# PythonOptimizers/pysparse

Measured on AMD Instinct MI355X. Metric: CSR SpMV GB/s (7-pt Poisson, % of 8 TB/s HBM peak) + PCG iters/s, higher is better.
Workload: dtype f64

## Files before the change

### include/pysparse_hip.h

```cpp
#ifndef PYSPARSE_HIP_H
#define PYSPARSE_HIP_H

#include <stddef.h>
#include <stdint.h>

#ifdef __cplusplus
extern "C" {
#endif

#define PSP_OK 0
#define PSP_EINVAL (-1)
#define PSP_ENODEV (-2)
#define PSP_ENOMEM (-3)
#define PSP_ESINGULAR (-4)
#define PSP_ECALLBACK (-5)

#define PSP_INFO_CONVERGED 0
#define PSP_INFO_MAXIT (-1)
#define PSP_INFO_ILLCOND_PRECON (-2)
#define PSP_INFO_NOT_SPD_PRECON (-3)
#define PSP_INFO_STAGNATION (-5)
#define PSP_INFO_BREAKDOWN (-6)

typedef struct psp_csr psp_csr_t;
// ... 1 lines not shown
typedef struct psp_jacobi psp_jacobi_t;
typedef struct psp_ssor psp_ssor_t;
typedef struct psp_op psp_op_t;


const char *psp_last_error(void);
const char *psp_version(void);
int psp_device_count(void);
int psp_set_device(int device);
int psp_thread_info(int *thread_slot, int *device, void **hip_stream);
int psp_debug_hold_handles(const void *h1, const void *h2, int milliseconds);
int psp_debug_mid_count(long long *solves, long long *fallbacks);
int psp_debug_brick_count(long long *solves, long long *fallbacks);
int psp_debug_shake(long long seed, int min_us, int max_us, unsigned point_mask, unsigned rank_mask, int revert_mask);
int psp_debug_shake_count(long long *injected);
int psp_debug_spin(int microseconds);
int psp_peer_access(int device, int peer, int *can_access);
int psp_set_placement(int on);
int psp_placement_info(int *enabled, long long *draws, double *draw_ms_total);
int psp_place_operands(const psp_csr_t *A, double **y_dev, double **x_dev, double *report6);
int psp_set_stream(void *hip_stream);
int psp_synchronize(void);
int psp_device_info(char *name, int name_len, int *compute_units, int64_t *hbm_bytes);
int psp_mem_info(int64_t *free_bytes, int64_t *total_bytes);

int psp_malloc(void **dev, size_t bytes);
int psp_free(void *dev);
int psp_memcpy_h2d(void *dev, const void *host, size_t bytes);
int psp_memcpy_d2h(void *host, const void *dev, size_t bytes);
int psp_memset(void *dev, int byte, size_t bytes);
int psp_trim(void);
int psp_event_create(void **event);
int psp_event_destroy(void *event);
int psp_event_record(void *event);
int psp_event_elapsed_ms(void *start, void *stop, float *ms);
int psp_stream_probe(int reads, int writes, size_t bytes_per_stream, int reps, float *avg_ms, float *min_ms);
int psp_last_solve_info(char *name, int name_cap, int *info);
int psp_set_single_kernel_loops(int on);
const char *psp_build_id(void);


int psp_csr_create(int nrows, int ncols, int nnz, const int *ind_host, const int *col_host,
                   const double *val_host, psp_csr_t **out);
int psp_csr_poisson(int nx, int ny, int nz, psp_csr_t **out);
int psp_csr_poisson_slab(int nx, int ny, int nz, int64_t row_lo, int64_t row_hi, int64_t col_shift,
                         int ncols_local, psp_csr_t **out);
int psp_csr_poisson_big(int nx, int ny, int nz, psp_csr_t **out);
int psp_csr_poisson_big_slab(int nx, int ny, int nz, int64_t row_lo, int64_t row_hi, int64_t col_shift,
                             int ncols_local, psp_csr_t **out);
int64_t psp_csr_nnz64(const psp_csr_t *A);
int psp_csr_poisson_multi(int nx, int ny, int nz, const int *devices, int ndev, psp_csr_t **out);
int psp_csr_create_multi(int nrows, int ncols, int nnz, const int *ind_host, const int *col_host,
                         const double *val_host, const int *devices, int ndev, psp_csr_t **out);
int psp_csr_multi_info(const psp_csr_t *A, int *nranks, int *distinct_devices, int *uses_rccl);
int psp_multi_plan(int nrows, int ncols, const int *ind_host, const int *col_host, int ndev, int rank,
                   int64_t *row_range_out, int *counts_out, int *ghost_ids, int ghost_cap, int *links, int links_cap,
                   int *col_local);
int psp_csr_multi_spmv_time(psp_csr_t *A, int warmup, int reps, double *ms_per_product);
int psp_csr_multi_phase_time(psp_csr_t *A, int what, int warmup, int reps, double *ms_per_rep);
int psp_csr_create64(int nrows, int ncols, int64_t nnz, const int64_t *ind_host, const int *col_host,
                     const double *val_host, psp_csr_t **out);
int psp_csr_random_banded(int nrows, int ncols, int m, int stride, uint64_t seed, psp_csr_t **out);
int psp_csr_download_rows(const psp_csr_t *A, int row_lo, int row_hi, int64_t *ind_host, int *col_host,
                          double *val_host);
int psp_csr_destroy(psp_csr_t *A);
int psp_csr_shape(const psp_csr_t *A, int *nrows, int *ncols, int *nnz);
int psp_csr_download(const psp_csr_t *A, int *ind_host, int *col_host, double *val_host);
int psp_csr_diagonal(const psp_csr_t *A, double *diag_host);

int psp_csr_matvec(psp_csr_t *A, const double *x_host, double *y_host);
int psp_csr_matvec_stride(psp_csr_t *A, const double *x_host, ptrdiff_t incx, double *y_host,
                          ptrdiff_t incy);
int psp_csr_matvec_transp(psp_csr_t *A, const double *x_host, double *y_host);
int psp_csr_matvec_transp_stride(psp_csr_t *A, const double *x_host, ptrdiff_t incx,
                                 double *y_host, ptrdiff_t incy);
int psp_csr_matvec_dev(psp_csr_t *A, const double *x_dev, double *y_dev);
int psp_csr_matvec_transp_dev(psp_csr_t *A, const double *x_dev, double *y_dev);
int psp_csr_set_variant(psp_csr_t *A, int variant);
int psp_csr_set_schedule(psp_csr_t *A, int strip_rows);
int psp_csr_kernel_info(psp_csr_t *A, char *name, int name_cap, int *info);
int psp_csr_prepare(psp_csr_t *A, long long expected_products);
int psp_csr_release_arrays(psp_csr_t *A);
int psp_csr_setup_info(psp_csr_t *A, double *info4);
int psp_csr_renumbering(psp_csr_t *A, int *perm_host, int *available);
int64_t psp_csr_device_bytes(const psp_csr_t *A);


int psp_sss_create(int n, int nnz_lower, const int *ind_host, const int *col_host,
                   const double *val_host, const double *diag_host, psp_sss_t **out);
int psp_sss_poisson(int nx, int ny, int nz, psp_sss_t **out);
int psp_sss_destroy(psp_sss_t *A);
int psp_sss_kernel_info(psp_sss_t *A, char *name, int name_cap, int *info);
int psp_sss_prepare(psp_sss_t *A, long long expected_products);
int psp_sss_setup_info(psp_sss_t *A, double *info4);
int psp_sss_set_variant(psp_sss_t *A, int variant);
int psp_sss_shape(const psp_sss_t *A, int *n, int *nnz_reported);
int psp_sss_download(const psp_sss_t *A, int *ind_host, int *col_host, double *val_host,
                     double *diag_host);
int psp_sss_getitem(const psp_sss_t *A, int i, int j, double *value);
int psp_sss_matvec(psp_sss_t *A, const double *x_host, double *y_host);
int psp_sss_matvec_stride(psp_sss_t *A, const double *x_host, ptrdiff_t incx, double *y_host,
                          ptrdiff_t incy);
int psp_sss_matvec_dev(psp_sss_t *A, const double *x_dev, double *y_dev);
int64_t psp_sss_device_bytes(const psp_sss_t *A);


int psp_jacobi_create_csr(psp_csr_t *A, double omega, int steps, psp_jacobi_t **out);
int psp_jacobi_create_sss(psp_sss_t *A, double omega, int steps, psp_jacobi_t **out);
int psp_jacobi_create_diag(int n, const double *diag_host, double omega, int steps,
                           const psp_op_t *A_or_null, psp_jacobi_t **out);
int psp_jacobi_destroy(psp_jacobi_t *K);
int psp_jacobi_shape(const psp_jacobi_t *K, int *n);
int psp_jacobi_precon(psp_jacobi_t *K, const double *x_host, double *y_host);
int psp_jacobi_precon_dev(psp_jacobi_t *K, const double *x_dev, double *y_dev);


int psp_ssor_create(psp_sss_t *A, double omega, int steps, psp_ssor_t **out);
int psp_ssor_destroy(psp_ssor_t *K);
int psp_ssor_info(const psp_ssor_t *K, int *n, int *levels_forward, int *levels_backward);
int psp_ssor_run_info(const psp_ssor_t *K, int *runs_forward, int *runs_backward, long *levels_in_runs,
                      long *slots_in_runs);
int psp_ssor_brick_info(const psp_ssor_t *K, int *bricks, int *edge);
int psp_ssor_precon(psp_ssor_t *K, const double *x_host, double *y_host);
int psp_ssor_precon_dev(psp_ssor_t *K, const double *x_dev, double *y_dev);


typedef int (*psp_host_apply_fn)(void *ctx, int n, const double *x_host, double *y_host);

int psp_op_from_csr(psp_csr_t *A, psp_op_t **out);
int psp_op_from_sss(psp_sss_t *A, psp_op_t **out);
int psp_op_from_jacobi(psp_jacobi_t *K, psp_op_t **out);
int psp_op_from_ssor(psp_ssor_t *K, psp_op_t **out);
int psp_op_from_callback(int n, psp_host_apply_fn fn, void *ctx, psp_op_t **out);
int psp_op_destroy(psp_op_t *op);


int psp_pcg(const psp_op_t *A, const psp_op_t *K, int n, double *x_host, const double *b_host,
            double tol, int maxit, int *info, int *iter, double *relres, double *hist_host);
int psp_pcg_dev(const psp_op_t *A, const psp_op_t *K, int n, double *x_dev, const double *b_dev,
                double tol, int maxit, int *info, int *iter, double *relres, double *hist_host);

int psp_minres(const psp_op_t *A, const psp_op_t *K, int n, double *x_host, const double *b_host,
               double tol, int maxit, int *info, int *iter, double *relres, double *hist_host);
int psp_minres_dev(const psp_op_t *A, const psp_op_t *K, int n, double *x_dev,
                   const double *b_dev, double tol, int maxit, int *info, int *iter,
                   double *relres, double *hist_host);

int psp_cgs(const psp_op_t *A, const psp_op_t *K, int n, double *x_host, const double *b_host,
            double tol, int maxit, int *info, int *iter, double *relres);
int psp_bicgstab(const psp_op_t *A, const psp_op_t *K, int n, double *x_host, const double *b_host,
                 double tol, int maxit, int *info, int *iter, double *relres);
int psp_qmrs(const psp_op_t *A, const psp_op_t *K, int n, double *x_host, const double *b_host,
             double tol, int maxit, int *info, int *iter, double *relres);
int psp_gmres(const psp_op_t *A, const psp_op_t *K, int n, double *x_host, const double *b_host,
              double tol, int maxit, int dim, int *info, int *iter, double *relres);


int psp_k_hint_constant(const double *v_dev, int n);
int psp_k_unhint(const double *v_dev);
int psp_k_dot(int n, const double *x_dev, const double *y_dev, double *out_dev);
int psp_k_residual(int n, const double *b_dev, double *r_dev, const double *dinv_dev,
                   double *out_dev);
int psp_k_pupdate(int n, const double *r_dev, const double *dinv_dev, double beta, int first,
                  double *p_dev);
int psp_k_csr_matvec_dot(psp_csr_t *A, const double *p_dev, int p_offset, double *q_dev,
                         double *out_dev);
// ... 67 lines not shown
```

### pysparse_amd/_capi.py

```python
import ctypes as C
import os

HERE = os.path.dirname(os.path.abspath(__file__))
LIB_PATH = os.environ.get("PSP_LIB_OVERRIDE") or os.path.join(HERE, "libpysparse_hip.so")

SYMBOLS = """
psp_last_error psp_version psp_device_count psp_set_device psp_thread_info psp_debug_hold_handles psp_debug_mid_count psp_debug_brick_count psp_debug_shake psp_debug_shake_count psp_debug_spin psp_peer_access psp_set_stream psp_synchronize
psp_set_placement psp_placement_info psp_place_operands psp_device_info psp_mem_info psp_malloc psp_free psp_memcpy_h2d psp_memcpy_d2h psp_memset psp_trim
psp_event_create psp_event_destroy psp_event_record psp_event_elapsed_ms psp_stream_probe psp_build_id psp_last_solve_info psp_set_single_kernel_loops
psp_csr_create psp_csr_poisson psp_csr_poisson_slab psp_csr_poisson_big psp_csr_poisson_big_slab psp_csr_nnz64 psp_csr_create64 psp_csr_random_banded psp_csr_download_rows psp_csr_destroy psp_csr_shape
psp_csr_download psp_csr_diagonal psp_csr_matvec psp_csr_matvec_stride psp_csr_matvec_transp
psp_csr_matvec_transp_stride psp_csr_matvec_dev psp_csr_matvec_transp_dev psp_csr_set_variant
psp_csr_set_schedule psp_csr_kernel_info psp_csr_prepare psp_csr_setup_info psp_csr_release_arrays psp_csr_renumbering psp_csr_device_bytes
psp_csr_poisson_multi psp_csr_create_multi psp_csr_multi_info psp_csr_multi_spmv_time psp_csr_multi_phase_time psp_multi_plan
psp_sss_create psp_sss_poisson psp_sss_destroy psp_sss_shape psp_sss_download psp_sss_getitem
psp_sss_matvec psp_sss_matvec_stride psp_sss_matvec_dev psp_sss_device_bytes
psp_sss_kernel_info psp_sss_set_variant psp_sss_prepare psp_sss_setup_info
psp_jacobi_create_csr psp_jacobi_create_sss psp_jacobi_create_diag psp_jacobi_destroy
psp_jacobi_shape psp_jacobi_precon psp_jacobi_precon_dev
psp_ssor_create psp_ssor_destroy psp_ssor_info psp_ssor_run_info psp_ssor_brick_info psp_ssor_precon psp_ssor_precon_dev
psp_op_from_csr psp_op_from_sss psp_op_from_jacobi psp_op_from_ssor psp_op_from_callback psp_op_destroy
psp_pcg psp_pcg_dev psp_minres psp_minres_dev psp_cgs psp_bicgstab psp_qmrs psp_gmres
psp_k_dot psp_k_residual psp_k_pupdate psp_k_csr_matvec_dot psp_k_xr_update psp_k_gather
psp_k_csr_matvec_overlap psp_k_hint_constant psp_k_unhint psp_k_px_update psp_k_r_update psp_k_x_update
psp_k_jacobi psp_pcgstate_create psp_pcgstate_destroy psp_pcgstate_init psp_pcgstate_fetch psp_pcgstate_hist
psp_kd_px_update psp_kd_csr_matvec_overlap psp_kd_pcg_scalar_xpq psp_kd_r_update psp_kd_pcg_scalar_r
psp_minresstate_create psp_minresstate_destroy psp_minresstate_init psp_minresstate_fetch psp_minresstate_hist
psp_kd_minres_scale psp_kd_minres_matvec psp_kd_minres_lanczos psp_kd_minres_scalar psp_kd_minres_wx
""".split()


class PcgStatus(C.Structure):
    _fields_ = [("status", C.c_int), ("info", C.c_int), ("iter", C.c_int), ("it", C.c_int), ("xpend", C.c_int),
                ("stag0", C.c_int), ("pend_maxit", C.c_int), ("relres", C.c_double), ("normr", C.c_double),
                ("n2b", C.c_double), ("alpha_x", C.c_double)]


class MinresStatus(C.Structure):
    _fields_ = [("status", C.c_int), ("stop", C.c_int), ("info", C.c_int), ("iter", C.c_int),
                ("relres", C.c_double), ("norm_rmr", C.c_double)]

WAIT_FN = C.CFUNCTYPE(C.c_int, C.c_void_p)
HOST_APPLY_FN = C.CFUNCTYPE(C.c_int, C.c_void_p, C.c_int, C.POINTER(C.c_double), C.POINTER(C.c_double))


class PspError(RuntimeError):
    def __init__(self, code, msg):
        RuntimeError.__init__(self, "libpysparse_hip error %d: %s" % (code, msg))
        self.code = code


_lib = None


def lib():
    global _lib
    if _lib is None:
        if not os.path.exists(LIB_PATH):
            raise ImportError("%s not found: run `python -c 'import __graft_entry__ as g; g.build()'` "
                              "(hipcc --offload-arch=gfx950); there is no CPU fallback" % LIB_PATH)
        L = C.CDLL(LIB_PATH)
        _declare(L)
        _lib = L
    return _lib


def check(rc):
    if rc != 0:
        raise PspError(rc, lib().psp_last_error().decode())
    return rc


def _declare(L):
    vp, i, d, i64 = C.c_void_p, C.c_int, C.c_double, C.c_int64
    pvp, pi, pd = C.POINTER(C.c_void_p), C.POINTER(C.c_int), C.POINTER(C.c_double)
    sz, pt = C.c_size_t, C.c_ssize_t
    L.psp_last_error.restype = C.c_char_p
    L.psp_last_error.argtypes = []
    L.psp_version.restype = C.c_char_p
    L.psp_version.argtypes = []
    L.psp_device_count.restype = i
    L.psp_device_count.argtypes = []
    sig = {
        "psp_set_device": [i], "psp_thread_info": [pi, pi, pvp], "psp_debug_hold_handles": [vp, vp, i], "psp_debug_shake": [C.c_longlong, i, i, C.c_uint, C.c_uint, i], "psp_debug_shake_count": [C.POINTER(C.c_longlong)], "psp_debug_spin": [i], "psp_debug_mid_count": [C.POINTER(C.c_longlong), C.POINTER(C.c_longlong)], "psp_debug_brick_count": [C.POINTER(C.c_longlong), C.POINTER(C.c_longlong)], "psp_peer_access": [i, i, pi], "psp_set_stream": [vp], "psp_synchronize": [], "psp_trim": [],
        "psp_set_placement": [i], "psp_placement_info": [pi, C.POINTER(C.c_longlong), pd], "psp_place_operands": [vp, pvp, pvp, pd],
        "psp_device_info": [C.c_char_p, i, pi, C.POINTER(i64)],
        "psp_mem_info": [C.POINTER(i64), C.POINTER(i64)],
        "psp_malloc": [pvp, sz], "psp_free": [vp], "psp_memcpy_h2d": [vp, vp, sz],
        "psp_memcpy_d2h": [vp, vp, sz], "psp_memset": [vp, i, sz],
        "psp_event_create": [pvp], "psp_event_destroy": [vp], "psp_event_record": [vp],
        "psp_event_elapsed_ms": [vp, vp, C.POINTER(C.c_float)],
        "psp_stream_probe": [i, i, sz, i, C.POINTER(C.c_float), C.POINTER(C.c_float)],
        "psp_csr_create": [i, i, i, vp, vp, vp, pvp],
        "psp_csr_poisson": [i, i, i, pvp], "psp_csr_poisson_big": [i, i, i, pvp],
        "psp_csr_poisson_slab": [i, i, i, i64, i64, i64, i, pvp],
        "psp_csr_poisson_big_slab": [i, i, i, i64, i64, i64, i, pvp],
        "psp_csr_create64": [i, i, i64, vp, vp, vp, pvp],
        "psp_csr_poisson_multi": [i, i, i, vp, i, pvp], "psp_csr_create_multi": [i, i, i, vp, vp, vp, vp, i, pvp],
        "psp_csr_multi_info": [vp, pi, pi, pi], "psp_csr_multi_spmv_time": [vp, i, i, pd], "psp_csr_multi_phase_time": [vp, i, i, i, pd],
        "psp_multi_plan": [i, i, vp, vp, i, i, C.POINTER(i64), vp, vp, i, vp, i, vp],
        "psp_csr_random_banded": [i, i, i, i, C.c_uint64, pvp],
        "psp_csr_download_rows": [vp, i, i, vp, vp, vp],
        "psp_csr_destroy": [vp], "psp_csr_shape": [vp, pi, pi, pi],
        "psp_csr_download": [vp, vp, vp, vp], "psp_csr_diagonal": [vp, vp],
        "psp_csr_matvec": [vp, vp, vp], "psp_csr_matvec_stride": [vp, vp, pt, vp, pt],
        "psp_csr_matvec_transp": [vp, vp, vp], "psp_csr_matvec_transp_stride": [vp, vp, pt, vp, pt],
        "psp_csr_matvec_dev": [vp, vp, vp], "psp_csr_matvec_transp_dev": [vp, vp, vp],
        "psp_csr_set_variant": [vp, i], "psp_csr_set_schedule": [vp, i],
        "psp_csr_kernel_info": [vp, C.c_char_p, i, pi],
        "psp_csr_renumbering": [vp, vp, pi],
        "psp_sss_create": [i, i, vp, vp, vp, vp, pvp], "psp_sss_poisson": [i, i, i, pvp],
        "psp_sss_destroy": [vp], "psp_sss_shape": [vp, pi, pi],
        "psp_sss_download": [vp, vp, vp, vp, vp], "psp_sss_getitem": [vp, i, i, pd],
        "psp_sss_matvec": [vp, vp, vp], "psp_sss_matvec_stride": [vp, vp, pt, vp, pt],
        "psp_sss_matvec_dev": [vp, vp, vp],
        "psp_sss_kernel_info": [vp, C.c_char_p, i, pi], "psp_sss_set_variant": [vp, i],
        "psp_jacobi_create_csr": [vp, d, i, pvp], "psp_jacobi_create_sss": [vp, d, i, pvp],
        "psp_jacobi_create_diag": [i, vp, d, i, vp, pvp], "psp_jacobi_destroy": [vp],
        "psp_jacobi_shape": [vp, pi], "psp_jacobi_precon": [vp, vp, vp],
        "psp_jacobi_precon_dev": [vp, vp, vp],
        "psp_ssor_create": [vp, d, i, pvp], "psp_ssor_destroy": [vp], "psp_ssor_info": [vp, pi, pi, pi], "psp_ssor_run_info": [vp, pi, pi, vp, vp], "psp_ssor_brick_info": [vp, pi, pi],
        "psp_ssor_precon": [vp, vp, vp], "psp_ssor_precon_dev": [vp, vp, vp], "psp_op_from_ssor": [vp, pvp],
        "psp_op_from_csr": [vp, pvp], "psp_op_from_sss": [vp, pvp], "psp_op_from_jacobi": [vp, pvp],
        "psp_op_from_callback": [i, HOST_APPLY_FN, vp, pvp], "psp_op_destroy": [vp],
        "psp_pcg": [vp, vp, i, vp, vp, d, i, pi, pi, pd, vp],
        "psp_pcg_dev": [vp, vp, i, vp, vp, d, i, pi, pi, pd, vp],
        "psp_minres": [vp, vp, i, vp, vp, d, i, pi, pi, pd, vp],
        "psp_minres_dev": [vp, vp, i, vp, vp, d, i, pi, pi, pd, vp],
        "psp_cgs": [vp, vp, i, vp, vp, d, i, pi, pi, pd], "psp_bicgstab": [vp, vp, i, vp, vp, d, i, pi, pi, pd],
        "psp_qmrs": [vp, vp, i, vp, vp, d, i, pi, pi, pd], "psp_gmres": [vp, vp, i, vp, vp, d, i, i, pi, pi, pd],
        "psp_k_dot": [i, vp, vp, vp], "psp_k_residual": [i, vp, vp, vp, vp],
        "psp_k_pupdate": [i, vp, vp, d, i, vp], "psp_k_csr_matvec_dot": [vp, vp, i, vp, vp],
        "psp_k_xr_update": [i, d, vp, vp, vp, vp, vp, vp], "psp_k_gather": [i, vp, vp, vp],
        "psp_k_csr_matvec_overlap": [vp, vp, i, vp, i, i, WAIT_FN, vp, vp],
        "psp_k_hint_constant": [vp, i], "psp_k_unhint": [vp],
        "psp_k_px_update": [i, vp, vp, d, i, d, i, vp, vp, vp], "psp_k_r_update": [i, d, vp, vp, vp, vp],
        "psp_k_x_update": [i, d, vp, vp, vp],
        "psp_k_jacobi": [i, vp, vp, vp],
        "psp_pcgstate_create": [pvp], "psp_pcgstate_destroy": [vp], "psp_pcgstate_init": [vp, d, d, d, d, i, i],
        "psp_pcgstate_fetch": [vp, C.POINTER(PcgStatus)], "psp_pcgstate_hist": [vp, i, i, vp],
        "psp_kd_px_update": [vp, i, vp, vp, vp, vp, vp],
        "psp_kd_csr_matvec_overlap": [vp, vp, vp, i, vp, i, i, WAIT_FN, vp, vp],
        "psp_kd_pcg_scalar_xpq": [vp, vp], "psp_kd_r_update": [vp, i, vp, vp, vp, vp],
        "psp_kd_pcg_scalar_r": [vp, vp],
        "psp_minresstate_create": [pvp], "psp_minresstate_destroy": [vp],
        "psp_minresstate_init": [vp, d, d, d, i, i], "psp_minresstate_fetch": [vp, C.POINTER(MinresStatus)],
        "psp_minresstate_hist": [vp, i, i, vp],
        "psp_kd_minres_scale": [vp, i, vp, vp],
        "psp_kd_minres_matvec": [vp, vp, vp, i, vp, i, i, WAIT_FN, vp, vp],
        "psp_kd_minres_lanczos": [vp, i, vp, vp, vp, vp, vp, vp], "psp_kd_minres_scalar": [vp, i, vp],
        "psp_kd_minres_wx": [vp, i, vp, vp, vp, vp],
        "psp_last_solve_info": [C.c_char_p, i, C.POINTER(i)], "psp_set_single_kernel_loops": [i],
        "psp_csr_release_arrays": [vp], "psp_csr_prepare": [vp, C.c_longlong], "psp_sss_prepare": [vp, C.c_longlong],
        "psp_csr_setup_info": [vp, C.POINTER(d)], "psp_sss_setup_info": [vp, C.POINTER(d)],
    }
    for name, argtypes in sig.items():
        f = getattr(L, name)
        f.restype = i
        f.argtypes = argtypes
    L.psp_build_id.restype = C.c_char_p
    L.psp_build_id.argtypes = []
    L.psp_csr_device_bytes.restype = i64
    L.psp_csr_device_bytes.argtypes = [vp]
    L.psp_csr_nnz64.restype = i64
    L.psp_csr_nnz64.argtypes = [vp]
    L.psp_sss_device_bytes.restype = i64
    L.psp_sss_device_bytes.argtypes = [vp]
```

### pysparse_amd/csrc/psp_csr_abi.h

```cpp

__global__ __launch_bounds__(256) void csr_validate_kernel(int nnz, int ncols, const int *__restrict__ col,
                                                           unsigned long long *bad) {
  for (long k = (long)blockIdx.x * 256 + threadIdx.x; k < nnz; k += (long)gridDim.x * 256) {
    const int c = col[k];
    if (c < 0 || c >= ncols) atomicMin(bad, (unsigned long long)k);
  }
}

extern "C" {

int psp_csr_create(int nrows, int ncols, int nnz, const int *ind_host, const int *col_host,
                   const double *val_host, psp_csr_t **out) {
  if (psp::cpu_mode()) return psp::cpu::csr_create(nrows, ncols, nnz, ind_host, col_host, val_host, out);
  if (!out || !ind_host || (nnz > 0 && (!col_host || !val_host)))
    return fail(PSP_EINVAL, "psp_csr_create: NULL argument");
  if (nrows < 0 || ncols < 0 || nnz < 0) return fail(PSP_EINVAL, "psp_csr_create: negative size");
  if (ind_host[0] != 0 || ind_host[nrows] != nnz)
    return fail(PSP_EINVAL, "psp_csr_create: ind[0] must be 0 and ind[nrows] == nnz");
  for (int i = 0; i < nrows; ++i)
    if (ind_host[i + 1] < ind_host[i])
      return fail(PSP_EINVAL, "psp_csr_create: ind not monotone at row %d", i);
  const bool check_on_device = nnz >= (1 << 22);
  if (!check_on_device)
    for (int k = 0; k < nnz; ++k)
// ... 231 lines not shown
    if (rc == PSP_OK) rc = finalize_csr(P);
    if (rc != PSP_OK) {
      if (P) psp_csr_destroy(P);
      if (A) psp_csr_destroy(A);
      return rc;
    }
    if (!A) {
      *out = P;
      return PSP_OK;
    }
    P->no_reorder = true;
    A->parts[p] = P;
    A->part_row0[p] = (int)r0;
    A->max_row_nnz = std::max(A->max_row_nnz, P->max_row_nnz);
  }
  A->part_row0[np] = nrows;
  *out = A;
  return PSP_OK;
}

int psp_csr_download_rows(const psp_csr_t *A, int row_lo, int row_hi, int64_t *ind_host, int *col_host,
                          double *val_host) {
  if (A && A->multi) return fail(PSP_EINVAL, "%s is not available on a multi-device matrix (psp_csr_*_multi): use matvec, jacobi, pcg, minres", "psp_csr_download_rows");
  if (!A || !ind_host) return fail(PSP_EINVAL, "psp_csr_download_rows: NULL argument");
  if (A->w4_only) return fail(PSP_EINVAL, "psp_csr_download_rows: the operator has no CSR arrays (psp_csr_poisson_big, psp_csr_release_arrays)");
  if (row_lo < 0 || row_hi > A->nrows || row_lo > row_hi) return fail(PSP_EINVAL, "psp_csr_download_rows: bad row range");
  int64_t written = 0;
  ind_host[0] = 0;
  const int np = A->nparts ? A->nparts : 1;
  for (int p = 0; p < np; ++p) {
    const psp_csr *P = A->nparts ? A->parts[p] : A;
    const int p0 = A->nparts ? A->part_row0[p] : 0;
    const int a = std::max(row_lo, p0) - p0, b = std::min(row_hi, p0 + P->nrows) - p0;
    if (a >= b) continue;
    std::vector<int> pi((size_t)(b - a) + 1);
    PSP_HIP(hipMemcpy(pi.data(), P->ind + a, sizeof(int) * pi.size(), hipMemcpyDeviceToHost));
    const int k0 = pi[0], cnt = pi.back() - k0;
    for (int r = a; r < b; ++r) ind_host[(size_t)(p0 + r - row_lo) + 1] = written + (pi[(size_t)(r - a) + 1] - k0);
    if (cnt > 0) {
      if (col_host) PSP_HIP(hipMemcpy(col_host + written, P->col + k0, sizeof(int) * (size_t)cnt, hipMemcpyDeviceToHost));
      if (val_host) PSP_HIP(hipMemcpy(val_host + written, P->val + k0, sizeof(double) * (size_t)cnt, hipMemcpyDeviceToHost));
    }
    written += cnt;
  }
  return PSP_OK;
}

int psp_csr_destroy(psp_csr_t *A) {
  if (!A) return PSP_OK;
  if (A->host) return psp::cpu::csr_destroy(A);
  if (A->multi) {
    PSP_API_GUARD_H(A);
    const int rc = psp::multi_destroy(A->multi);
    delete A;
    return rc;
  }
  psp_csr *transposed = nullptr, *reordered = nullptr;
  {
    std::lock_guard<std::mutex> lk(g_extra_mu);
    auto it = g_extra.find(A);
    if (it != g_extra.end()) {
      transposed = it->second.transposed;
      reordered = it->second.reordered;
      if (it->second.perm) (void)hipFree(it->second.perm);
      if (it->second.inv) (void)hipFree(it->second.inv);
      if (it->second.xp) (void)hipFree(it->second.xp);
      for (auto &t : it->second.t) {
        if (t.second.tab) (void)hipFree(t.second.tab);
        if (t.second.rowoff) (void)hipFree(t.second.rowoff);
        if (t.second.blist) (void)hipFree(t.second.blist);
        if (t.second.blist6) (void)hipFree(t.second.blist6);
        if (t.second.col16) (void)hipFree(t.second.col16);
        if (t.second.ulist) (void)hipFree(t.second.ulist);
        if (t.second.colu) (void)hipFree(t.second.colu);
        if (t.second.perm) (void)hipFree(t.second.perm);
      }
      if (it->second.big_partials) (void)hipFree(it->second.big_partials);
      if (it->second.packed) (void)hipFree(it->second.packed);
      if (it->second.dia_val) (void)hipFree(it->second.dia_val);
      if (it->second.dia_mask) (void)hipFree(it->second.dia_mask);
      if (it->second.dia_mask32) (void)hipFree(it->second.dia_mask32);
      if (it->second.dia_mask64) (void)hipFree(it->second.dia_mask64);
      if (it->second.dia_offs_dev) (void)hipFree(it->second.dia_offs_dev);
      g_extra.erase(it);
    }
  }
  for (int p = 0; p < A->nparts; ++p) psp_csr_destroy(A->parts[p]);
  delete[] A->parts;
  delete[] A->part_row0;
  if (transposed) psp_csr_destroy(transposed);
  if (reordered) psp_csr_destroy(reordered);
  (void)hipFree(A->ind);
  (void)hipFree(A->col);
  (void)hipFree(A->val);
  delete A;
  return PSP_OK;
}

int psp_csr_shape(const psp_csr_t *A, int *nrows, int *ncols, int *nnz) {
  if (!A) return fail(PSP_EINVAL, "psp_csr_shape: NULL handle");
  if (nrows) *nrows = A->nrows;
  if (ncols) *ncols = A->ncols;
  if (nnz) *nnz = A->nnz;
  return PSP_OK;
}

int psp_csr_download(const psp_csr_t *A, int *ind_host, int *col_host, double *val_host) {
  if (A && A->host) return psp::cpu::csr_download(A, ind_host, col_host, val_host);
  if (A && A->multi) return fail(PSP_EINVAL, "%s is not available on a multi-device matrix (psp_csr_*_multi): use matvec, jacobi, pcg, minres", "psp_csr_download");
  if (!A) return fail(PSP_EINVAL, "psp_csr_download: NULL handle");
  if (A->w4_only) return fail(PSP_EINVAL, "psp_csr_download: the operator has no CSR arrays (psp_csr_poisson_big, psp_csr_release_arrays)");
  if (A->nparts) return fail(PSP_EINVAL, "psp_csr_download: more than 2^31 nonzeros: use psp_csr_download_rows");
  if (ind_host)
    PSP_HIP(hipMemcpyAsync(ind_host, A->ind, sizeof(int) * ((size_t)A->nrows + 1),
                           hipMemcpyDeviceToHost, stream()));
  if (col_host && A->nnz)
    PSP_HIP(hipMemcpyAsync(col_host, A->col, sizeof(int) * (size_t)A->nnz, hipMemcpyDeviceToHost,
                           stream()));
  if (val_host && A->nnz)
    PSP_HIP(hipMemcpyAsync(val_host, A->val, sizeof(double) * (size_t)A->nnz,
                           hipMemcpyDeviceToHost, stream()));
  PSP_HIP(hipStreamSynchronize(stream()));
  return PSP_OK;
}

int psp_csr_diagonal_dev(const psp_csr_t *A, double *diag_dev) {
  PSP_API_GUARD_H(A);
  if (A && A->multi) return fail(PSP_EINVAL, "%s is not available on a multi-device matrix (psp_csr_*_multi): use matvec, jacobi, pcg, minres", "psp_csr_diagonal_dev");
  if (A->nrows == 0) return PSP_OK;
  if (A->nparts) {
    for (int p = 0; p < A->nparts; ++p) {
      const psp_csr *P = A->parts[p];
      if (P->nrows == 0) continue;
      hipLaunchKernelGGL(csr_diag_kernel, dim3(std::min((P->nrows + 255) / 256, 4096)), dim3(256), 0, stream(),
                         P->nrows, A->part_row0[p], P->ind, P->col, P->val, diag_dev + A->part_row0[p]);
    }
    PSP_LAUNCH_CHECK();
    return PSP_OK;
  }
  if (A->w4_only) {
    psp::CsrExtra *ex;
    PSP_TRY(ensure_w4(A, &ex));
    const int zero_slot = A->w4_diag_slot;
    hipLaunchKernelGGL(dia_diag_kernel, dim3(std::min((A->nrows + 255) / 256, 65536)), dim3(256), 0, stream(),
                       A->nrows, ex->dia_no, zero_slot, ex->dia_val, ex->dia_mask, diag_dev);
    PSP_LAUNCH_CHECK();
    return PSP_OK;
  }
  int grid = std::min((A->nrows + 255) / 256, 4096);
  hipLaunchKernelGGL(csr_diag_kernel, dim3(grid), dim3(256), 0, stream(), A->nrows, 0, A->ind, A->col,
                     A->val, diag_dev);
  PSP_LAUNCH_CHECK();
  return PSP_OK;
}

int psp_csr_diagonal(const psp_csr_t *A, double *diag_host) {
  PSP_API_GUARD_H(A);
  if (!A || !diag_host) return fail(PSP_EINVAL, "psp_csr_diagonal: NULL argument");
  if (A->host) return psp::cpu::csr_diagonal(A, diag_host);
  if (A->multi) return psp::multi_diagonal_host(A->multi, diag_host);
  DevBuf d;
  PSP_TRY(d.alloc(A->nrows));
  PSP_TRY(psp_csr_diagonal_dev(A, d.p));
  return download_strided(diag_host, d.p, A->nrows, 1);
}

// ... 96 lines not shown
      dperm = it->second.perm;
      on_device = it->second.reorder_on_device;
    }
  }
  if (!dperm) return PSP_OK;
  PSP_HIP(hipMemcpy(perm_host, dperm, sizeof(int) * (size_t)A->nrows, hipMemcpyDeviceToHost));
  *available = on_device ? 2 : 1;
  return PSP_OK;
}

int psp_csr_release_arrays(psp_csr_t *A) {
  PSP_API_GUARD_H(A);
  if (!A) return fail(PSP_EINVAL, "psp_csr_release_arrays: NULL handle");
  if (A->w4_only) return PSP_OK;
  if (A->host || A->multi || A->nparts || A->sym_owner)
    return fail(PSP_EINVAL, "psp_csr_release_arrays: not available for this kind of handle");
  PSP_TRY(ensure_device());
  psp::CsrExtra *ex;
  PSP_TRY(ensure_w4(A, &ex));
  if (ex->dia_state != 1 || ex->dia_no > 16)
    return fail(PSP_EINVAL, "psp_csr_release_arrays: the operator does not multiply with the index-free layout (csr_spmv_w4, "
                            "<= 16 offsets): its CSR arrays are what it streams");
  PSP_HIP(hipStreamSynchronize(stream()));
  int slot = -1;
  for (int o = 0; o < ex->dia_no; ++o)
    if (ex->dia_offs.o[o] == 0) slot = o;
  psp_csr *transposed = nullptr, *reordered = nullptr;
  {
    std::lock_guard<std::mutex> lk(g_extra_mu);
    transposed = ex->transposed;
    reordered = ex->reordered;
    ex->transposed = ex->reordered = nullptr;
    for (auto &t : ex->t) {
      if (t.second.tab) (void)hipFree(t.second.tab);
      if (t.second.rowoff) (void)hipFree(t.second.rowoff);
      if (t.second.blist) (void)hipFree(t.second.blist);
      if (t.second.blist6) (void)hipFree(t.second.blist6);
      if (t.second.col16) (void)hipFree(t.second.col16);
      if (t.second.ulist) (void)hipFree(t.second.ulist);
      if (t.second.colu) (void)hipFree(t.second.colu);
      if (t.second.perm) (void)hipFree(t.second.perm);
    }
    ex->t.clear();
    if (ex->packed) (void)hipFree(ex->packed);
    ex->packed = nullptr;
  }
  if (transposed) psp_csr_destroy(transposed);
  if (reordered) psp_csr_destroy(reordered);
  if (A->ind) (void)hipFree(A->ind);
  if (A->col) (void)hipFree(A->col);
  if (A->val) (void)hipFree(A->val);
  A->ind = A->col = nullptr;
  A->val = nullptr;
  A->padded = 0;
  A->nnz64 = A->nnz;
  A->w4_diag_slot = slot;
  A->max_row_nnz = ex->dia_no;
  A->variant = -1;
  A->w4_only = true;
  return PSP_OK;
}

int psp_csr_prepare(psp_csr_t *A, long long expected_products) {
  PSP_API_GUARD_H(A);
  if (!A) return fail(PSP_EINVAL, "psp_csr_prepare: NULL handle");
  if (A->host || A->multi || A->nparts) return PSP_OK;
  std::lock_guard<std::mutex> lk(g_extra_mu);
  g_extra[A].expected_products = expected_products < 0 ? 0 : (expected_products > 0x7fffffffffffLL ? 0x7fffffffffffLL : (long)expected_products);
  return PSP_OK;
}

int psp_csr_setup_info(psp_csr_t *A, double *info4) {
  PSP_API_GUARD_H(A);
  if (!A || !info4) return fail(PSP_EINVAL, "psp_csr_setup_info: NULL argument");
  info4[0] = info4[1] = info4[2] = info4[3] = 0.0;
  if (A->host || A->multi || A->nparts) return PSP_OK;
  std::lock_guard<std::mutex> lk(g_extra_mu);
  auto it = g_extra.find(A);
  if (it == g_extra.end()) return PSP_OK;
  info4[0] = it->second.reorder_ms;
  info4[1] = (double)it->second.products;
  info4[2] = (double)reorder_after();
  info4[3] = (double)it->second.reorder_state;
  return PSP_OK;
}

int psp_csr_kernel_info(psp_csr_t *A, char *name, int name_cap, int *info) {
  PSP_API_GUARD_H(A);
  if (!A) return fail(PSP_EINVAL, "psp_csr_kernel_info: NULL handle");
  if (A->host) {
    if (name && name_cap > 0) snprintf(name, name_cap, "cpu loops (PSP_DEVICE=cpu)");
    if (info) info[0] = info[1] = info[2] = info[3] = 0;
    return PSP_OK;
  }
  if (A->multi) {
    char buf[160];
    psp::multi_describe(A->multi, buf, sizeof buf);
    if (name && name_cap > 0) snprintf(name, name_cap, "%s", buf);
    if (info) info[0] = info[1] = info[2] = info[3] = 0;
    return PSP_OK;
  }
  if (A->nparts) return psp_csr_kernel_info(A->parts[0], name, name_cap, info);
  Variant v = decode_variant(A->variant);
  if (A->w4_only) v.w4 = true;
  const char *k = "csr_spmv_stream";
  int vals[4] = {0, 0, 0, 0};
  bool w4 = false;
  if (v.w4 && A->sym_owner) {
    psp_sss *S = const_cast<psp_sss *>(A->sym_owner);
    PSP_TRY(ensure_sss_w4(S));
    if (S->w4_state == 1) {
      w4 = true;
      k = "sss_spmv_w4";
      vals[0] = S->w4_nol;
    }
  }
  if (!w4 && v.w4) {
    psp::CsrExtra *ex;
    PSP_TRY(ensure_w4(A, &ex));
    if (ex->dia_state == 1) {
      w4 = true;
      k = "csr_spmv_w4";
      vals[0] = ex->dia_no;
    }
  }
  if (!w4 && A->nrows > 0 && (v.wave || v.w1) && A->max_row_nnz <= v.tile / 2) {
    k = v.wave ? "csr_spmv_wave" : "csr_spmv_w1";
    if (v.w2) {
      ChunkTable *t;
      PSP_TRY(get_chunk_table(A, v.tile, &t));
      PSP_TRY(ensure_rowoff(A, t));
      if (t->np != 0) {
        k = "csr_spmv_w2";
        if (v.w3) {
          PSP_TRY(ensure_w3(A, t));
          vals[1] = t->max_blocks;
          {
            psp::CsrExtra *exs = nullptr;
            int mode = 0;
            PSP_TRY(pick_scattered(A, t, &exs, &mode));
            if (mode == 1) {
              ChunkTable *rt;
              PSP_TRY(get_chunk_table(exs->reordered, 1024, &rt));
              k = "csr_spmv_w3_rcm";
              vals[0] = rt->nb;
              vals[1] = rt->max_blocks;
              vals[3] = t->max_blocks;
            } else if (mode == 2) {
              k = "csr_spmv_w5";
              vals[0] = t->nu;
              vals[3] = t->max_cols;
            }
          }
          if (t->nb > 0) {
            k = "csr_spmv_w3";
            vals[0] = t->nb;
            if (v.sched) {
              PSP_TRY(ensure_schedule(A, t));
              vals[2] = t->sched_state == 1;
              vals[3] = t->half_band;
            }
          }
        }
        if (v.w6 && !strcmp(k, "csr_spmv_w2")) {
          PSP_TRY(ensure_w6(A, t));
          if (t->nb6 > 0) {
// ... 351 lines not shown
```

### pysparse_amd/csrc/psp_csr_kernels.h

```cpp

constexpr int kBlock = 256;


__global__ void build_chunk_table(int nrows, const int *__restrict__ ind, int target, int nchunks,
                                  int2 *__restrict__ tab) {
  int c = blockIdx.x * blockDim.x + threadIdx.x;
  if (c > nchunks) return;
  int r;
  if (c == nchunks) {
    r = nrows;
  } else {
    long want = (long)c * target;
    int lo = 0, hi = nrows;
    while (lo < hi) {
      int mid = lo + ((hi - lo) >> 1);
      if ((long)ind[mid] >= want)
        hi = mid;
      else
        lo = mid + 1;
    }
    r = lo;
  }
  tab[c] = make_int2(r, ind[r]);
}
// ... 1255 lines not shown
      if constexpr (NTS)
        __builtin_nontemporal_store(outu, reinterpret_cast<d2u *>(y + r));
      else
        *reinterpret_cast<d2u *>(y + r) = outu;
      if (dotv) {
        d2u u;
        if (dot_slot >= 0) {
          u.x = 0.0;
          u.y = 0.0;
#pragma unroll
          for (int o = 0; o < NO; ++o)
            if (o == dot_slot) {
              u.x = xv[o].x;
              u.y = xv[o].y;
            }
        } else {
          u = *reinterpret_cast<const d2u *>(dotv + r);
          if (use_div) {
            u.x = u.x / xdiv;
            u.y = u.y / xdiv;
          }
        }
        dsum += u.x * a0;
        dsum += u.y * a1;
      }
    } else {
      y[r] = a0;
      if (dotv) {
        double u0 = 0.0;
        if (dot_slot >= 0) {
#pragma unroll
          for (int o = 0; o < NO; ++o)
            if (o == dot_slot) u0 = xv[o].x;
        } else {
          u0 = use_div ? dotv[r] / xdiv : dotv[r];
        }
        dsum += u0 * a0;
      }
    }
  }
  if (partials) {
    dsum = wave_sum(dsum);
    if (lane == 0) red[wid] = dsum;
    __syncthreads();
    if (threadIdx.x == 0) partials[blockIdx.x] = red[0] + red[1] + red[2] + red[3];
  }
}

struct SssOffs {
  int o[8];
};

__global__ void sss_lowmask_kernel(int n, int nol, SssOffs offs, const int *__restrict__ ind,
                                   const int *__restrict__ col, const double *__restrict__ val,
                                   double *__restrict__ valL, unsigned char *__restrict__ low, long soa_npad) {
  for (long r = (long)blockIdx.x * blockDim.x + threadIdx.x; r < n; r += (long)gridDim.x * blockDim.x) {
    const long blk = r / kDiaRows;
    const int i = (int)(r % kDiaRows);
    unsigned m = 0;
    for (int k = ind[r]; k < ind[r + 1]; ++k) {
      const int o = col[k] - (int)r;
      int b = 0;
      while (b < nol - 1 && offs.o[b] != o) ++b;
      m |= 1u << b;
      if (soa_npad > 0) valL[(size_t)b * soa_npad + r] = val[k];
      else valL[((size_t)blk * nol + b) * kDiaRows + i] = val[k];
    }
    low[r] = (unsigned char)m;
  }
}

__global__ void sss_mask_kernel(int n, int nol, SssOffs offs, const unsigned char *__restrict__ low,
                                unsigned short *__restrict__ mask) {
  for (long r = (long)blockIdx.x * blockDim.x + threadIdx.x; r < n; r += (long)gridDim.x * blockDim.x) {
    unsigned m = low[r];
    for (int j = 0; j < nol; ++j) {
      const long ru = r - offs.o[j];
      if (ru < n && ((low[ru] >> j) & 1u)) m |= 1u << (8 + j);
    }
    mask[r] = (unsigned short)m;
  }
}

template <int NOL, int FLAGS = 0>
__global__ __launch_bounds__(256) void sss_spmv_w4(
    int n, int stripe, SssOffs offs, const double *__restrict__ valL, const double *__restrict__ diag,
    const unsigned short *__restrict__ mask, const double *__restrict__ x, double *__restrict__ y,
    const double *__restrict__ dotv, double *__restrict__ partials, const int *__restrict__ skip,
    int use_div, double xdiv, const double *__restrict__ xdiv_dev, int dot_is_x) {
  if (skip && *skip) return;
  if (xdiv_dev) xdiv = *xdiv_dev;
  __shared__ double red[4];
  const int lane = threadIdx.x & 63;
  const int wid = __builtin_amdgcn_readfirstlane(threadIdx.x >> 6);
  int vb = (int)blockIdx.x;
  if (stripe > 0) {
    const int k = vb >> 3;
    vb = ((k / stripe) * 8 + (vb & 7)) * stripe + k % stripe;
  }
  const long blk = (long)vb * 4 + wid;
  const long r = blk * kDiaRows + 2 * lane;
  double dsum = 0.0;
  if (r < n) {
    const bool two = r + 1 < n;
    const unsigned mm = *reinterpret_cast<const unsigned *>(mask + r);
    const unsigned m0 = mm & 0xffffu, m1 = mm >> 16;
    const long npad = ((long)n + kDiaRows - 1) / kDiaRows * kDiaRows;
    const long xmax = (long)n - 2;
    bool edge = !two;
    constexpr bool SOA = (FLAGS & 8) != 0;
    auto vaddr = [&](long row, int j) -> const double * {
      return SOA ? valL + (size_t)j * npad + row
                 : valL + ((size_t)(row / kDiaRows) * NOL + j) * kDiaRows + (size_t)(row % kDiaRows);
    };
    d2v vl[NOL], xl[NOL];
    constexpr bool SHFL = (FLAGS & 4) != 0;
    const bool off1 = SHFL && offs.o[NOL - 1] == -1;
#pragma unroll
    for (int j = 0; j < NOL; ++j) {
      vl[j] = ldg<(FLAGS & 1) != 0>(reinterpret_cast<const d2v *>(vaddr(r, j)));
      if (off1 && j == NOL - 1) continue;
      const long c = r + offs.o[j];
      const long cc = c < 0 ? 0 : c;
      const d2u t = *reinterpret_cast<const d2u *>(x + cc);
      xl[j].x = t.x;
      xl[j].y = t.y;
      edge |= c < 0;
    }
    double halo_xm1 = 0.0, halo_x2 = 0.0, halo_v2 = 0.0;
    if (off1) {
      if (lane == 0 && r > 0) halo_xm1 = x[r - 1];
      if (lane == 63) {
        if (r + 2 < n) halo_x2 = x[r + 2];
        if (r + 2 < npad)
          halo_v2 = *vaddr(r + 2, NOL - 1);
      }
    }
    d2v dg, x0;
    {
      const long rd = r > xmax ? xmax : r;
      const d2u t = *reinterpret_cast<const d2u *>(diag + rd);
      const d2u u = *reinterpret_cast<const d2u *>(x + rd);
      dg.x = t.x; dg.y = t.y; x0.x = u.x; x0.y = u.y;
    }
    d2v vu[NOL], xu[NOL];
#pragma unroll
    for (int j = 0; j < NOL; ++j) {
      if (off1 && j == NOL - 1) continue;
      const long ru = r - offs.o[j];
      if (SHFL && (offs.o[j] & 1) == 0) {
        const long v0 = ru < npad ? ru : npad - 2;
        vu[j] = ldg<(FLAGS & 2) != 0>(reinterpret_cast<const d2v *>(vaddr(v0, j)));
      } else {
        const long v0 = ru < npad ? ru : npad - 1, v1 = ru + 1 < npad ? ru + 1 : npad - 1;
        vu[j].x = ldg<(FLAGS & 2) != 0>(vaddr(v0, j));
        vu[j].y = ldg<(FLAGS & 2) != 0>(vaddr(v1, j));
      }
      const long xr = ru > xmax ? xmax : ru;
      const d2u t = *reinterpret_cast<const d2u *>(x + xr);
      xu[j].x = t.x;
      xu[j].y = t.y;
      edge |= ru > xmax;
    }
    if (edge) {
#pragma unroll
      for (int j = 0; j < NOL; ++j) {
        const long c = r + offs.o[j];
        if (c < 0) {
          xl[j].x = 0.0;
          xl[j].y = c + 1 >= 0 ? x[c + 1] : 0.0;
        }
        const long ru = r - offs.o[j];
        if (ru > xmax) {
          xu[j].x = ru < n ? x[ru] : 0.0;
          xu[j].y = 0.0;
        }
      }
      if (!two) {
        dg.x = diag[r];
        dg.y = 0.0;
        x0.x = x[r];
        x0.y = 0.0;
      }
    }
    if (off1) {
      constexpr int j = NOL - 1;
      const double up = __shfl_up(x0.y, 1, 64);
      const double dnx = __shfl_down(x0.x, 1, 64);
      const double dnv = __shfl_down(vl[j].x, 1, 64);
      xl[j].x = lane == 0 ? halo_xm1 : up;
      xl[j].y = x0.x;
      vu[j].x = vl[j].y;
      vu[j].y = lane == 63 ? halo_v2 : dnv;
      xu[j].x = x0.y;
      xu[j].y = lane == 63 ? halo_x2 : dnx;
    }
    if (use_div) {
#pragma unroll
      for (int j = 0; j < NOL; ++j) {
        xl[j].x = xl[j].x / xdiv;
        xl[j].y = xl[j].y / xdiv;
        xu[j].x = xu[j].x / xdiv;
        xu[j].y = xu[j].y / xdiv;
      }
      x0.x = x0.x / xdiv;
      x0.y = x0.y / xdiv;
    }
    double a0 = 0.0, a1 = 0.0;
#pragma unroll
    for (int j = 0; j < NOL; ++j) {
      const double t0 = a0 + vl[j].x * xl[j].x;
      const double t1 = a1 + vl[j].y * xl[j].y;
      a0 = ((m0 >> j) & 1u) ? t0 : a0;
      a1 = ((m1 >> j) & 1u) ? t1 : a1;
    }
    a0 = a0 + dg.x * x0.x;
    a1 = a1 + dg.y * x0.y;
#pragma unroll
    for (int j = NOL - 1; j >= 0; --j) {
      const double t0 = a0 + vu[j].x * xu[j].x;
      const double t1 = a1 + vu[j].y * xu[j].y;
      a0 = ((m0 >> (8 + j)) & 1u) ? t0 : a0;
      a1 = ((m1 >> (8 + j)) & 1u) ? t1 : a1;
    }
    if (two) {
      d2u outu;
      outu.x = a0;
      outu.y = a1;
      __builtin_nontemporal_store(outu, reinterpret_cast<d2u *>(y + r));
      if (dotv) {
        d2u u;
        if (dot_is_x) {
          u.x = x0.x;
          u.y = x0.y;
        } else {
          u = *reinterpret_cast<const d2u *>(dotv + r);
          if (use_div) {
            u.x = u.x / xdiv;
            u.y = u.y / xdiv;
          }
        }
        dsum += u.x * a0;
        dsum += u.y * a1;
      }
    } else {
      y[r] = a0;
      if (dotv) dsum += (dot_is_x ? x0.x : (use_div ? dotv[r] / xdiv : dotv[r])) * a0;
    }
  }
  if (partials) {
    dsum = wave_sum(dsum);
    if (lane == 0) red[wid] = dsum;
    __syncthreads();
    if (threadIdx.x == 0) partials[blockIdx.x] = red[0] + red[1] + red[2] + red[3];
  }
}

template <int NO>
__global__ __launch_bounds__(256) void csr_spmv_w4x(
    int blk0, int blk1, int nrows, int ncols, int stripe, DiaOffs offs, const double *__restrict__ valT,
    const unsigned *__restrict__ mask, const double *__restrict__ x, double *__restrict__ y,
    const double *__restrict__ dotv, double *__restrict__ partials, const int *__restrict__ skip) {
  if (skip && *skip) return;
  __shared__ double red[4];
  const int lane = threadIdx.x & 63;
  const int wid = __builtin_amdgcn_readfirstlane(threadIdx.x >> 6);
  int vb = (int)blockIdx.x;
  if (stripe > 0) {
    const int k = vb >> 3;
    vb = ((k / stripe) * 8 + (vb & 7)) * stripe + k % stripe;
  }
  const int blk = blk0 + vb * 4 + wid;
  const long r = (long)blk * kDiaRows + 2 * lane;
  double dsum = 0.0;
  if (blk < blk1 && r < nrows) {
    const uint2 mm = *reinterpret_cast<const uint2 *>(mask + r);
    const unsigned m0 = mm.x, m1 = mm.y;
    const double *vp = valT + (size_t)blk * NO * kDiaRows + 2 * lane;
    const long cmax = (long)ncols - 2;
    double a0 = 0.0, a1 = 0.0;
#pragma unroll
    for (int g = 0; g < NO; g += 8) {
      constexpr int G = 8;
      d2v v[G], xv[G];
      bool edge = false;
#pragma unroll
      for (int u = 0; u < G; ++u) {
        if (g + u < NO) {
          v[u] = ldg<true>(reinterpret_cast<const d2v *>(vp + (g + u) * kDiaRows));
          const long c = r + offs.o[g + u];
          const long cc = c < 0 ? 0 : (c > cmax ? cmax : c);
          const d2u t = *reinterpret_cast<const d2u *>(x + cc);
          xv[u].x = t.x;
          xv[u].y = t.y;
          edge |= cc != c;
        }
      }
      if (edge) {
#pragma unroll
        for (int u = 0; u < G; ++u) {
          if (g + u < NO) {
            const long c = r + offs.o[g + u];
            if (c < 0 || c > cmax) {
              xv[u].x = (c >= 0 && c < ncols) ? x[c] : 0.0;
              xv[u].y = (c + 1 >= 0 && c + 1 < ncols) ? x[c + 1] : 0.0;
            }
          }
        }
      }
#pragma unroll
      for (int u = 0; u < G; ++u) {
        if (g + u < NO) {
          const double t0 = a0 + v[u].x * xv[u].x;
          const double t1 = a1 + v[u].y * xv[u].y;
          a0 = ((m0 >> (g + u)) & 1u) ? t0 : a0;
          a1 = ((m1 >> (g + u)) & 1u) ? t1 : a1;
        }
      }
    }
    if (r + 1 < nrows) {
      d2u outu;
      outu.x = a0;
      outu.y = a1;
      __builtin_nontemporal_store(outu, reinterpret_cast<d2u *>(y + r));
      if (dotv) {
        const d2u u = *reinterpret_cast<const d2u *>(dotv + r);
        dsum += u.x * a0;
        dsum += u.y * a1;
      }
    } else {
      y[r] = a0;
      if (dotv) dsum += dotv[r] * a0;
    }
  }
  if (partials) {
    dsum = wave_sum(dsum);
    if (lane == 0) red[wid] = dsum;
// ... 415 lines not shown
```

### pysparse_amd/csrc/psp_csr_select.h

```cpp
namespace psp {

static int colmask() {
#ifdef PSP_TUNING
  static const int m = [] {
    const char *e = psp::tuning_env("PSP_SPMV_COLMASK");
    return e ? atoi(e) : -1;
  }();
  return m;
#else
  return -1;
#endif
}

static int spmv_stripe() {
  static const int m = [] {
    const char *e = psp::tuning_env("PSP_SPMV_STRIPE");
    return e ? atoi(e) : -1;
  }();
  return m;
}

static int w4_auto_stripe(const psp_csr *A) {
  if (A->sym_owner) return 32;
  int plane_wgs = 0;
// ... 94 lines not shown
}

static void launch_w5(const psp_csr *A, const ChunkTable *t, int grid, int stripe, int c0, int c1, const double *x,
                      double *y, const double *dotv, double *pbuf, const int *skip) {
  if (t->np == 2) launch_w5_np<2>(A, t, grid, stripe, c0, c1, x, y, dotv, pbuf, skip);
  else if (t->np == 3) launch_w5_np<3>(A, t, grid, stripe, c0, c1, x, y, dotv, pbuf, skip);
  else launch_w5_np<4>(A, t, grid, stripe, c0, c1, x, y, dotv, pbuf, skip);
}

constexpr long kReorderAfter = 2048;
static long reorder_after() {
  static const long v = [] {
    const char *e = psp::tuning_env("PSP_SPMV_REORDER_AFTER");
    return e ? atol(e) : kReorderAfter;
  }();
  return v;
}

static int pick_scattered(const psp_csr *A, ChunkTable *t, psp::CsrExtra **ex_out, int *mode, bool count = false) {
  *mode = 0;
  if (t->nb != 0 || t->max_blocks <= 0) return PSP_OK;
  const int var = A->variant < 0 ? 0 : A->variant;
  if (((var >> 27) & 1) == 0) {
    psp::CsrExtra *exr;
    bool due;
    {
      std::lock_guard<std::mutex> lk(g_extra_mu);
      exr = &g_extra[A];
      due = exr->reorder_state >= 0 || exr->products >= reorder_after() || exr->expected_products >= reorder_after();
      if (count && !due) exr->products += 1;
    }
    if (due) {
      PSP_TRY(ensure_reordered(A, exr, t->max_blocks));
      if (exr->reorder_state == 1) {
        *ex_out = exr;
        *mode = 1;
        return PSP_OK;
      }
    }
  }
  if (((var >> 28) & 1) == 0) {
    PSP_TRY(ensure_w5(A, t));
    if (t->nu > 0) *mode = 2;
  }
  return PSP_OK;
}

static int launch_reordered(const psp_csr *A, psp::CsrExtra *ex, int stripe, const double *x, double *y,
                            const double *dotv, double *partials, int *nparts, const int *skip) {
  psp_csr *R = ex->reordered;
  ChunkTable *t;
  PSP_TRY(get_chunk_table(R, 1024, &t));
  int grid = (t->nchunks + 3) / 4;
  if (stripe > 0) grid = (grid + 8 * stripe - 1) / (8 * stripe) * (8 * stripe);
  const int n = A->nrows;
  double *xp = ex->xp, *yp = ex->xp + n;
  static const bool gather_form = [] {
    const char *e = psp::tuning_env("PSP_SPMV_REORDER_GATHER");
    return e && atoi(e) != 0;
  }();
  if (gather_form) PSP_TRY(psp::reorder_gather(n, ex->perm, x, xp, skip));
  else PSP_TRY(psp::reorder_scatter(n, ex->inv, x, xp, skip));
  R->variant = A->variant;
  launch_w3(R, t, true, grid, stripe, 0, t->nchunks, xp, yp, nullptr, nullptr, skip);
  PSP_LAUNCH_CHECK();
  const int gback = (n + 1023) / 1024;
  double *pbuf = partials;
  if (partials && gback > kMaxParts) {
    PSP_TRY(ensure_big_partials(ex, gback));
    pbuf = ex->big_partials;
  }
  int np = 0;
  if (!partials && !gather_form) PSP_TRY(psp::reorder_scatter(n, ex->perm, yp, y, skip));
  else PSP_TRY(psp::reorder_back(n, ex->inv, yp, y, partials ? dotv : nullptr, pbuf, &np, skip));
  if (partials && pbuf != partials) {
    hipLaunchKernelGGL(fold_partials_kernel, dim3(kFold / 16), dim3(256), 0, stream(), pbuf, np, partials, kFold);
    PSP_LAUNCH_CHECK();
    np = kFold;
  }
  if (nparts) *nparts = np;
  return PSP_OK;
}

int csr_spmv_scaled_launch(const psp_csr *A, const double *x, double xdiv, double *y, double *partials,
                           int *nparts, int *available, const int *skip, const double *xdiv_dev) {
  *available = 0;
  static const bool on = [] {
    const char *e = psp::tuning_env("PSP_MINRES_SCALED");
    return e ? atoi(e) != 0 : true;
  }();
  Variant v = decode_variant(A->variant);
  if (A->w4_only) v.w4 = true;
  if (!on || !v.w4 || A->nparts || A->nrows != A->ncols || A->nrows < 2) return PSP_OK;
  const int stripe = w4_stripe(A, v);
  const int nblk = (A->nrows + kDiaRows - 1) / kDiaRows;
  const int grid = w4_grid(nblk, stripe);
  psp::CsrExtra *ex;
  {
    std::lock_guard<std::mutex> lk(g_extra_mu);
    ex = &g_extra[A];
  }
  bool sss = false;
  if (A->sym_owner) {
    psp_sss *S = const_cast<psp_sss *>(A->sym_owner);
    PSP_TRY(ensure_sss_w4(S));
    sss = S->w4_state == 1;
  }
  if (!sss) {
    PSP_TRY(ensure_w4(A, &ex));
    if (ex->dia_state != 1 || ex->dia_no > 16) return PSP_OK;
  }
  double *pbuf = partials;
  if (partials && grid > kMaxParts) {
    PSP_TRY(ensure_big_partials(ex, grid));
    pbuf = ex->big_partials;
  }
  if (sss)
    PSP_TRY(launch_sss_w4(A->sym_owner, stripe, x, y, x, pbuf, skip, grid, 1, xdiv, xdiv_dev));
  else
    PSP_TRY(launch_w4(A, ex, stripe, 0, nblk, x, y, x, pbuf, skip, grid, 1, xdiv, xdiv_dev));
  int np = grid;
  if (pbuf != partials) {
    np = kFold;
    hipLaunchKernelGGL(fold_partials_kernel, dim3(np / 16), dim3(256), 0, stream(), pbuf, grid, partials, np);
    PSP_LAUNCH_CHECK();
  }
  if (nparts) *nparts = np;
  *available = 1;
  return PSP_OK;
}

__global__ __launch_bounds__(256) void grid_wrap_check_kernel(int n, int nx, int ny, const unsigned short *__restrict__ mask,
                                                              int *__restrict__ bad) {
  int found = 0;
  for (long r = (long)blockIdx.x * blockDim.x + threadIdx.x; r < n; r += (long)gridDim.x * blockDim.x) {
    const unsigned m = mask[r];
    const int i = (int)(r % nx), j = (int)((r / nx) % ny);
    if (((m >> 2) & 1u) && i == 0) found = 1;
    if (((m >> 4) & 1u) && i == nx - 1) found = 1;
    if (((m >> 1) & 1u) && j == 0) found = 1;
    if (((m >> 5) & 1u) && j == ny - 1) found = 1;
  }
  if (found) atomicAdd(bad, 1);
}

__global__ __launch_bounds__(256) void w4_value_range_kernel(int n, int no, const double *__restrict__ valT,
                                                             const unsigned short *__restrict__ mask, double *__restrict__ out) {
  __shared__ double smin[4][16], smax[4][16];
  double lo[16], hi[16];
  for (int o = 0; o < 16; ++o) {
    lo[o] = INFINITY;
    hi[o] = -INFINITY;
  }
  for (long r = (long)blockIdx.x * blockDim.x + threadIdx.x; r < n; r += (long)gridDim.x * blockDim.x) {
    const unsigned m = mask[r];
    const double *vp = valT + (size_t)(r / kDiaRows) * no * kDiaRows + (size_t)(r % kDiaRows);
    for (int o = 0; o < no; ++o)
      if ((m >> o) & 1u) {
        const double v = vp[(size_t)o * kDiaRows];
        lo[o] = v < lo[o] ? v : lo[o];
        hi[o] = v > hi[o] ? v : hi[o];
        if (!(v == v)) hi[o] = INFINITY, lo[o] = -INFINITY;
      }
  }
  const int lane = threadIdx.x & 63, wid = threadIdx.x >> 6;
  for (int o = 0; o < no; ++o) {
    double a = lo[o], b = hi[o];
    for (int off = 32; off > 0; off >>= 1) {
      const double a2 = __shfl_down(a, off, 64), b2 = __shfl_down(b, off, 64);
      a = a2 < a ? a2 : a;
      b = b2 > b ? b2 : b;
    }
    if (lane == 0) {
      smin[wid][o] = a;
      smax[wid][o] = b;
    }
  }
  __syncthreads();
  if ((int)threadIdx.x < no) {
    const int o = threadIdx.x;
    double a = smin[0][o], b = smax[0][o];
    for (int w = 1; w < 4; ++w) {
      a = smin[w][o] < a ? smin[w][o] : a;
      b = smax[w][o] > b ? smax[w][o] : b;
    }
    out[((size_t)blockIdx.x * no + o) * 2] = a;
    out[((size_t)blockIdx.x * no + o) * 2 + 1] = b;
  }
}

int csr_w4_view(const psp_csr *A, W4View *out, int *available) {
  *available = 0;
  Variant v = decode_variant(A->variant);
  if (A->w4_only) v.w4 = true;
  if (!v.w4 || A->nparts || A->multi || A->host || A->nrows != A->ncols || A->nrows < 2) return PSP_OK;
  psp::CsrExtra *ex;
  PSP_TRY(ensure_w4(A, &ex));
  if (ex->dia_state != 1 || ex->dia_no > 9 || !ex->dia_mask) return PSP_OK;
  out->no = ex->dia_no;
  for (int i = 0; i < 12; ++i) out->offs[i] = i < ex->dia_no ? ex->dia_offs.o[i] : 0;
  out->valT = ex->dia_val;
// ... 179 lines not shown
  return t->np != 0;
}

int csr_reordered_view(const psp_csr *A, psp_csr **R, const int **perm, const int **inv) {
  *R = nullptr;
  psp::setup_mark(nullptr);
  Variant v = decode_variant(A->variant);
  if (A->nparts || A->w4_only || A->no_reorder || !(v.w1 && v.w2 && v.w3) || A->nrows != A->ncols ||
      A->max_row_nnz > v.tile / 2 || v.tile != 1024)
    return PSP_OK;
  if (v.w4) {
    if (A->sym_owner) {
      psp_sss *S = const_cast<psp_sss *>(A->sym_owner);
      PSP_TRY(ensure_sss_w4(S));
      if (S->w4_state == 1) return PSP_OK;
    }
    psp::CsrExtra *ex;
    PSP_TRY(ensure_w4(A, &ex));
    if (ex->dia_state == 1) return PSP_OK;
  }
  psp::setup_mark("first use: index-free (w4) layouts tried");
  ChunkTable *t;
  PSP_TRY(get_chunk_table(const_cast<psp_csr *>(A), v.tile, &t));
  PSP_TRY(ensure_rowoff(A, t));
  if (t->np == 0) return PSP_OK;
  psp::setup_mark("first use: chunk table + row offsets");
  PSP_TRY(ensure_w3(A, t));
  psp::setup_mark("first use: w3 tables on the stored numbering");
  psp::CsrExtra *exs = nullptr;
  int mode = 0;
  PSP_TRY(pick_scattered(A, t, &exs, &mode));
  if (mode != 1) return PSP_OK;
  exs->reordered->variant = A->variant;
  *R = exs->reordered;
  *perm = exs->perm;
  *inv = exs->inv;
  return PSP_OK;
}

int csr_spmv_launch(const psp_csr *A, const double *x, double *y, const double *dotv,
                    double *partials, int *nparts, const int *skip) {
  Workspace *w;
  PSP_TRY(workspace(&w));
  psp::setup_mark(nullptr);
  if (A->nparts) {
    double *tmp = w->partials + (size_t)(kSlots - 1) * kMaxParts;
    if (partials && (partials == tmp || (long)A->nparts * kFold > kMaxParts))
      return fail(PSP_EINVAL, "csr_spmv_launch: partitioned matrix needs a partial-sum slot other than the last");
    for (int p = 0; p < A->nparts; ++p) {
      const psp_csr *P = A->parts[p];
      if (P->nrows == 0) continue;
      const int r0 = A->part_row0[p];
      int np = 0;
      PSP_TRY(csr_spmv_launch(P, x, y + r0, (partials && dotv) ? dotv + r0 : nullptr, partials ? tmp : nullptr, &np,
                              skip));
      if (partials) {
        hipLaunchKernelGGL(fold_partials_kernel, dim3(kFold / 16), dim3(256), 0, stream(), tmp, np,
                           partials + (size_t)p * kFold, kFold);
        PSP_LAUNCH_CHECK();
      }
    }
    if (nparts) *nparts = A->nparts * kFold;
    return PSP_OK;
  }
  Variant v = decode_variant(A->variant);
  if (A->w4_only) v.w4 = true;
  if (v.w4 && A->sym_owner) {
    psp_sss *S = const_cast<psp_sss *>(A->sym_owner);
    PSP_TRY(ensure_sss_w4(S));
    if (S->w4_state == 1) {
      const int stripe = w4_stripe(A, v);
      const int nblk = (S->n + kDiaRows - 1) / kDiaRows;
      const int grid = w4_grid(nblk, stripe);
      double *pbuf = partials;
      if (partials && grid > kMaxParts) {
        psp::CsrExtra *ex;
        {
          std::lock_guard<std::mutex> lk(g_extra_mu);
          ex = &g_extra[A];
        }
        PSP_TRY(ensure_big_partials(ex, grid));
        pbuf = ex->big_partials;
      }
      PSP_TRY(launch_sss_w4(S, stripe, x, y, dotv, pbuf, skip, grid));
      int np = grid;
      if (pbuf != partials) {
        np = kFold;
        hipLaunchKernelGGL(fold_partials_kernel, dim3(np / 16), dim3(256), 0, stream(), pbuf, grid,
                           partials, np);
        PSP_LAUNCH_CHECK();
      }
      if (nparts) *nparts = np;
      return PSP_OK;
    }
  }
  if (v.w4) {
    psp::CsrExtra *ex;
    PSP_TRY(ensure_w4(A, &ex));
    if (ex->dia_state == 1) {
      const int stripe = w4_stripe(A, v);
      const int nblk = (A->nrows + kDiaRows - 1) / kDiaRows;
      const int grid = w4_grid(nblk, stripe);
      double *pbuf = partials;
      if (partials && grid > kMaxParts) {
        PSP_TRY(ensure_big_partials(ex, grid));
        pbuf = ex->big_partials;
      }
      PSP_TRY(launch_w4(A, ex, stripe, 0, nblk, x, y, dotv, pbuf, skip, grid));
      int np = grid;
      if (pbuf != partials) {
        np = kFold;
        hipLaunchKernelGGL(fold_partials_kernel, dim3(np / 16), dim3(256), 0, stream(), pbuf, grid,
                           partials, np);
        PSP_LAUNCH_CHECK();
      }
      if (nparts) *nparts = np;
      return PSP_OK;
    }
  }
  if (A->w4_only) return fail(PSP_EINVAL, "this operator exists only in the w4 layout (psp_csr_poisson_big)");
  if ((v.wave || v.w1) && A->max_row_nnz > v.tile / 2) {
    v.wave = v.w1 = v.w2 = false;
    v.tile = 2048;
    v.vec = 4;
    v.map_mode = 0;
    v.full_grid = false;
  }
  ChunkTable *t;
  PSP_TRY(get_chunk_table(const_cast<psp_csr *>(A), v.tile, &t));
  if (v.w1) {
    if (v.w3) v.wpb = 4;
    if (v.w2 && (v.full_grid || v.nt || v.layout == 1)) v.wpb = 4;
    int grid = (t->nchunks + v.wpb - 1) / v.wpb;
    const int stripe = spmv_stripe() >= 0 ? spmv_stripe() : v.stripe;
    if (stripe > 0) grid = (grid + 8 * stripe - 1) / (8 * stripe) * (8 * stripe);
    if (v.w2) {
      PSP_TRY(ensure_rowoff(A, t));
      if (t->np == 0) v.w2 = false;
    }
    bool use_w3 = false;
    const int *perm = nullptr;
    if (v.w2 && v.w3) {
      PSP_TRY(ensure_w3(A, t));
      use_w3 = t->nb > 0;
      if (use_w3 && v.sched) {
        PSP_TRY(ensure_schedule(A, t));
        if (t->sched_state == 1) {
          perm = t->perm;
          grid = t->sched_grid;
        }
      }
    }
    double *pbuf = partials;
    psp::CsrExtra *ex = nullptr;
    if (partials && grid > kMaxParts) {
      std::lock_guard<std::mutex> lk(g_extra_mu);
      ex = &g_extra[A];
      if (ex->big_cap < grid) {
        if (ex->big_partials) (void)hipFree(ex->big_partials);
        ex->big_partials = nullptr;
        ex->big_cap = 0;
        PSP_HIP(hipMalloc((void **)&ex->big_partials, sizeof(double) * (size_t)grid));
        ex->big_cap = grid;
      }
      pbuf = ex->big_partials;
    }
    if (!use_w3 && v.w2 && v.w3) {
// ... 511 lines not shown
```

### pysparse_amd/csrc/psp_csr_tables.h

```cpp

struct ChunkTable {
  int tile = 0;
  int target = 0;
  int nchunks = 0;
  int2 *tab = nullptr;
  int max_rows = -1;
  int np = 0;
  unsigned short *rowoff = nullptr;
  int nb = -1;
  int max_blocks = 0;
  int outliers = 0;
  int *blist = nullptr;
  unsigned short *col16 = nullptr;
  int nb6 = -1;
  int direct6 = 0;
  int *blist6 = nullptr;
  int nu = -1;
  int max_cols = 0;
  int *ulist = nullptr;
  unsigned short *colu = nullptr;
  int sched_state = -1;
  int sched_grid = 0;
  int *perm = nullptr;
  int half_band = 0;
};
static int get_chunk_table(psp_csr *A, int tile, ChunkTable **out);

namespace psp {

struct SplitInfo {
  int tile, ca, cb;
};

struct CsrExtra {
  std::map<int, ChunkTable> t;
  std::map<std::pair<int, int>, SplitInfo> split;
  double *big_partials = nullptr;
  int big_cap = 0;
  char *packed = nullptr;
  int dia_state = -1;
  int dia_no = 0;
  DiaOffs dia_offs;
  double *dia_val = nullptr;
  unsigned short *dia_mask = nullptr;
  unsigned *dia_mask32 = nullptr;
  unsigned long long *dia_mask64 = nullptr;
  int *dia_offs_dev = nullptr;
  psp_csr *transposed = nullptr;
  int reorder_state = -1;
  long products = 0;
  long expected_products = 0;
  double reorder_ms = 0.0;
  psp_csr *reordered = nullptr;
  int *perm = nullptr;
  int *inv = nullptr;
  double *xp = nullptr;
  int orig_max_blocks = 0;
  bool reorder_on_device = false;
  int grid_state = -1;
  int grid_nx = 0, grid_ny = 0;
  int constv_state = -1;
  double constv[16] = {0};
};

}

#include <mutex>
#include <unordered_map>
static std::unordered_map<const psp_csr *, psp::CsrExtra> g_extra;
static std::mutex g_extra_mu;

static int finalize_csr(psp_csr *A) {
  int *d_max;
  PSP_HIP(hipMalloc((void **)&d_max, sizeof(int)));
  PSP_HIP(hipMemsetAsync(d_max, 0, sizeof(int), stream()));
  if (A->nrows > 0) {
    int grid = std::min((A->nrows + 255) / 256, 2048);
    hipLaunchKernelGGL(max_row_kernel, dim3(grid), dim3(256), 0, stream(), A->nrows, A->ind, d_max);
    PSP_LAUNCH_CHECK();
  }
  PSP_HIP(hipMemcpyAsync(&A->max_row_nnz, d_max, sizeof(int), hipMemcpyDeviceToHost, stream()));
  PSP_HIP(hipStreamSynchronize(stream()));
  PSP_HIP(hipFree(d_max));
  return PSP_OK;
}

static int get_chunk_table(psp_csr *A, int tile, ChunkTable **out) {
  std::lock_guard<std::mutex> lk(g_extra_mu);
  psp::CsrExtra &ex = g_extra[A];
  ChunkTable &t = ex.t[tile];
  if (t.tab == nullptr) {
    int target = (tile - A->max_row_nnz) & ~3;
    if (target < tile / 2) target = tile / 2;
    long nch = ((long)A->nnz + target - 1) / target;
    if (nch < 1) nch = 1;
    t.tile = tile;
    t.target = target;
    t.nchunks = (int)nch;
    PSP_HIP(hipMalloc((void **)&t.tab, sizeof(int2) * (nch + 1)));
    int grid = (int)((nch + 1 + 255) / 256);
    hipLaunchKernelGGL(build_chunk_table, dim3(grid), dim3(256), 0, stream(), A->nrows, A->ind,
                       target, (int)nch, t.tab);
    PSP_LAUNCH_CHECK();
  }
  *out = &t;
  return PSP_OK;
}

static int ensure_rowoff(const psp_csr *A, ChunkTable *t) {
  std::lock_guard<std::mutex> lk(g_extra_mu);
  if (t->max_rows >= 0) return PSP_OK;
  int *d_max;
  PSP_HIP(hipMalloc((void **)&d_max, sizeof(int)));
  PSP_HIP(hipMemsetAsync(d_max, 0, sizeof(int), stream()));
  hipLaunchKernelGGL(max_chunk_rows_kernel, dim3(std::min((t->nchunks + 255) / 256, 2048)), dim3(256),
                     0, stream(), t->nchunks, t->tab, d_max);
  PSP_LAUNCH_CHECK();
  int mr = 0;
  PSP_HIP(hipMemcpyAsync(&mr, d_max, sizeof(int), hipMemcpyDeviceToHost, stream()));
  PSP_HIP(hipStreamSynchronize(stream()));
  PSP_HIP(hipFree(d_max));
  t->max_rows = mr;
  const int np = (mr + 1 + 63) / 64;
  if (np > 4) {
    t->np = 0;
    return PSP_OK;
  }
  const int npp = np < 2 ? 2 : np;
  const size_t entries = (size_t)t->nchunks * 64 * npp;
  PSP_HIP(hipMalloc((void **)&t->rowoff, sizeof(unsigned short) * entries));
  const int grid = (int)((entries + 255) / 256);
  if (npp == 2)
    hipLaunchKernelGGL(build_rowoff_kernel<2>, dim3(grid), dim3(256), 0, stream(), t->nchunks, t->target, t->tab, A->ind, t->rowoff);
  else if (npp == 3)
    hipLaunchKernelGGL(build_rowoff_kernel<3>, dim3(grid), dim3(256), 0, stream(), t->nchunks, t->target, t->tab, A->ind, t->rowoff);
  else
    hipLaunchKernelGGL(build_rowoff_kernel<4>, dim3(grid), dim3(256), 0, stream(), t->nchunks, t->target, t->tab, A->ind, t->rowoff);
  PSP_LAUNCH_CHECK();
  t->np = npp;
  return PSP_OK;
}

struct ScratchDev {
  void *p = nullptr;
  ~ScratchDev() {
// ... 391 lines not shown
  int grid = (nblocks + 3) / 4;
  if (stripe > 0) grid = (grid + 8 * stripe - 1) / (8 * stripe) * (8 * stripe);
  return grid;
}

static int ensure_big_partials(psp::CsrExtra *ex, int cap) {
  std::lock_guard<std::mutex> lk(g_extra_mu);
  if (ex->big_cap < cap) {
    if (ex->big_partials) (void)hipFree(ex->big_partials);
    ex->big_partials = nullptr;
    ex->big_cap = 0;
    PSP_HIP(hipMalloc((void **)&ex->big_partials, sizeof(double) * (size_t)cap));
    ex->big_cap = cap;
  }
  return PSP_OK;
}

static std::mutex g_sss_mu;
static int ensure_sss_w4(psp_sss *S) {
  std::lock_guard<std::mutex> lk(g_sss_mu);
  if (S->w4_state >= 0) return PSP_OK;
  S->w4_state = 0;
  static const bool off = [] {
    const char *e = psp::tuning_env("PSP_SSS_W4");
    return e && atoi(e) == 0;
  }();
  if (off || S->n < 2 || S->nnz_lower < 1) return PSP_OK;
  ScratchDev tab_mem;
  PSP_HIP(hipMalloc(&tab_mem.p, (kDiaTable + 1) * sizeof(int)));
  int *d_tab = (int *)tab_mem.p;
  int init[kDiaTable + 1];
  for (int i = 0; i < kDiaTable; ++i) init[i] = kDiaEmpty;
  init[kDiaTable] = 0;
  PSP_HIP(hipMemcpyAsync(d_tab, init, sizeof(init), hipMemcpyHostToDevice, stream()));
  hipLaunchKernelGGL(dia_offsets_kernel, dim3(std::min((S->n + 255) / 256, 8192)), dim3(256), 0, stream(), S->n,
                     S->ind, S->col, d_tab, d_tab + kDiaTable);
  PSP_LAUNCH_CHECK();
  int tab[kDiaTable + 1];
  PSP_HIP(hipMemcpyAsync(tab, d_tab, sizeof(tab), hipMemcpyDeviceToHost, stream()));
  PSP_HIP(hipStreamSynchronize(stream()));
  if (tab[kDiaTable]) return PSP_OK;
  std::vector<int> offs;
  for (int i = 0; i < kDiaTable; ++i)
    if (tab[i] != kDiaEmpty) offs.push_back(tab[i]);
  if (offs.empty() || offs.size() > 8) return PSP_OK;
  std::sort(offs.begin(), offs.end());
  const int nol = (int)offs.size();
  const size_t nblk = ((size_t)S->n + kDiaRows - 1) / kDiaRows;
  if ((double)nblk * kDiaRows * nol * 8.0 > 11.0 * (double)S->nnz_lower) return PSP_OK;
  SssOffs so;
  for (int i = 0; i < 8; ++i) so.o[i] = i < nol ? offs[i] : -1;
  const size_t nval = nblk * kDiaRows * nol;
  unsigned char *low = nullptr;
  hipError_t e1 = hipMalloc((void **)&S->w4_val, sizeof(double) * nval);
  hipError_t e2 = hipMalloc((void **)&S->w4_mask, sizeof(unsigned short) * (nblk * kDiaRows + 2));
  hipError_t e3 = hipMalloc((void **)&low, (size_t)S->n);
  if (e1 != hipSuccess || e2 != hipSuccess || e3 != hipSuccess) {
    (void)hipGetLastError();
    if (e1 == hipSuccess) (void)hipFree(S->w4_val);
    if (e2 == hipSuccess) (void)hipFree(S->w4_mask);
    if (e3 == hipSuccess) (void)hipFree(low);
    S->w4_val = nullptr;
    S->w4_mask = nullptr;
    return PSP_OK;
  }
  PSP_HIP(hipMemsetAsync(S->w4_val, 0, sizeof(double) * nval, stream()));
  PSP_HIP(hipMemsetAsync(S->w4_mask, 0, sizeof(unsigned short) * (nblk * kDiaRows + 2), stream()));
  const int grid = std::min((S->n + 255) / 256, 65536);
  bool soa = false;
  if (const char *e = psp::tuning_env("PSP_SSS_SOA")) soa = atoi(e) != 0;
  S->w4_soa = soa;
  hipLaunchKernelGGL(sss_lowmask_kernel, dim3(grid), dim3(256), 0, stream(), S->n, nol, so, S->ind, S->col,
                     S->val, S->w4_val, low, soa ? (long)(nblk * kDiaRows) : 0L);
  hipLaunchKernelGGL(sss_mask_kernel, dim3(grid), dim3(256), 0, stream(), S->n, nol, so, low, S->w4_mask);
  PSP_LAUNCH_CHECK();
  PSP_HIP(hipStreamSynchronize(stream()));
  PSP_HIP(hipFree(low));
  for (int i = 0; i < 8; ++i) S->w4_offs[i] = so.o[i];
  S->w4_nol = nol;
  S->w4_state = 1;
  return PSP_OK;
}

static int launch_sss_w4(const psp_sss *S, int stripe, const double *x, double *y, const double *dotv,
                         double *pbuf, const int *skip, int grid, int use_div = 0, double xdiv = 1.0,
                         const double *xdiv_dev = nullptr) {
  SssOffs so;
  for (int i = 0; i < 8; ++i) so.o[i] = S->w4_offs[i];
  const int flags = (S->full->variant >= 0 ? S->full->variant : 0) >> 23 & 3;
#define PSP_SW4_F(NOL, F)                                                                            \
  hipLaunchKernelGGL((sss_spmv_w4<NOL, F>), dim3(grid), dim3(256), 0, stream(), S->n, stripe, so,     \
                     S->w4_val, S->diag, S->w4_mask, x, y, dotv, pbuf, skip, use_div, xdiv, xdiv_dev,         \
                     (dotv == x && !w4_dot_reload()) ? 1 : 0)
  static const bool shfl = [] {
    const char *e = psp::tuning_env("PSP_SSS_SHFL");
    return e ? atoi(e) != 0 : true;
  }();
#define PSP_SW4(NOL)                                                                                 \
  case NOL:                                                                                          \
    if (S->w4_soa) PSP_SW4_F(NOL, 12);                                                               \
    else if (flags == 0 && shfl) PSP_SW4_F(NOL, 4);                                                  \
    else if (flags == 0) PSP_SW4_F(NOL, 0);                                                          \
    else if (flags == 1) PSP_SW4_F(NOL, 1);                                                          \
    else if (flags == 2) PSP_SW4_F(NOL, 2);                                                          \
    else PSP_SW4_F(NOL, 3);                                                                          \
    break
  switch (S->w4_nol) {
    PSP_SW4(1); PSP_SW4(2); PSP_SW4(3); PSP_SW4(4); PSP_SW4(5); PSP_SW4(6); PSP_SW4(7); PSP_SW4(8);
    default:
      return fail(PSP_EINVAL, "sss_spmv_w4: %d offsets", S->w4_nol);
  }
#undef PSP_SW4
#undef PSP_SW4_F
  PSP_LAUNCH_CHECK();
  return PSP_OK;
}

static int launch_w4_transp(const psp_csr *A, const double *x, double *y, int *available) {
  *available = 0;
  if (A->nparts) return PSP_OK;
  Variant v = decode_variant(A->variant);
  if (A->w4_only) v.w4 = true;
  if (!v.w4 || A->nrows < 1 || A->ncols < 1) return PSP_OK;
  psp::CsrExtra *ex;
  PSP_TRY(ensure_w4(A, &ex));
  if (ex->dia_state != 1 || ex->dia_no > 16) return PSP_OK;
  const int grid = (int)(((long)A->ncols + 511) / 512);
#define PSP_W4T(NO)                                                                                 \
  case NO:                                                                                          \
    hipLaunchKernelGGL((csr_spmv_w4_transp<NO>), dim3(grid), dim3(256), 0, stream(), A->nrows, A->ncols, \
                       ex->dia_offs, ex->dia_val, ex->dia_mask, x, y);                               \
    break
  switch (ex->dia_no) {
    PSP_W4T(1); PSP_W4T(2); PSP_W4T(3); PSP_W4T(4); PSP_W4T(5); PSP_W4T(6); PSP_W4T(7); PSP_W4T(8);
    PSP_W4T(9); PSP_W4T(10); PSP_W4T(11); PSP_W4T(12); PSP_W4T(13); PSP_W4T(14); PSP_W4T(15); PSP_W4T(16);
    default:
      return PSP_OK;
  }
#undef PSP_W4T
  PSP_LAUNCH_CHECK();
  *available = 1;
  return PSP_OK;
}

static int transpose_into(int nrows, int ncols, int nnz, const int *ind, const int *col, const double *val,
                          psp_csr *T) {
  int rc = PSP_OK;
  int *rows = nullptr, *pos = nullptr, *keys = nullptr, *perm = nullptr;
  void *tmp = nullptr;
#define TR_HIP(call)                                                                       \
  do {                                                                                     \
    hipError_t e_ = (call);                                                                \
    if (e_ != hipSuccess) {                                                                \
      rc = fail(e_ == hipErrorOutOfMemory ? PSP_ENOMEM : PSP_ENODEV, "%s: %s", #call,       \
                hipGetErrorString(e_));                                                    \
      goto done;                                                                           \
    }                                                                                      \
  } while (0)
  static const bool by_sort = [] {
    const char *e = psp::tuning_env("PSP_TRANSPOSE_SORT");
    return e && atoi(e) != 0;
  }();
  if (nnz > 0 && !by_sort) {
    double *kbuf = nullptr, *cbuf = nullptr;
    const size_t nk = (size_t)nnz, ncur = ((size_t)ncols + 3) / 2 + 1;
    constexpr int kTranspMaxColumn = 4096;
    bool too_long = false;
    rc = psp::scratch_get(nk, &kbuf);
    if (rc == PSP_OK) rc = psp::scratch_get(ncur, &cbuf);
    if (rc == PSP_OK) {
      unsigned long long *key = reinterpret_cast<unsigned long long *>(kbuf);
      int *cursor = reinterpret_cast<int *>(cbuf);
      size_t bytes = 0;
      hipError_t e = hipMemsetAsync(cursor, 0, sizeof(int) * ((size_t)ncols + 3), stream());
      const int g = (int)std::min<long>(((long)nnz + 255) / 256, 65536);
      if (e == hipSuccess) {
        hipLaunchKernelGGL(transp_count_kernel, dim3(g), dim3(256), 0, stream(), nnz, ncols, col, cursor, cursor + ncols + 1);
        e = hipcub::DeviceScan::ExclusiveSum(nullptr, bytes, cursor, T->ind, ncols + 1, stream());
      }
      if (e == hipSuccess) e = hipMalloc(&tmp, bytes ? bytes : 1);
      if (e == hipSuccess) e = hipcub::DeviceScan::ExclusiveSum(tmp, bytes, cursor, T->ind, ncols + 1, stream());
      int flags[2] = {0, 0};
      if (e == hipSuccess) {
        hipLaunchKernelGGL(transp_maxlen_kernel, dim3(std::min((ncols + 255) / 256, 4096)), dim3(256), 0, stream(), ncols, T->ind,
                           cursor + ncols + 2);
        e = hipMemcpyAsync(flags, cursor + ncols + 1, sizeof(flags), hipMemcpyDeviceToHost, stream());
      }
      if (e == hipSuccess) e = hipStreamSynchronize(stream());
      const int bad = flags[0];
      too_long = flags[1] > kTranspMaxColumn;
      if (e == hipSuccess && bad) rc = fail(PSP_EINVAL, "transpose: a column index is out of range");
      if (e == hipSuccess && !bad && !too_long) e = hipMemsetAsync(cursor, 0, sizeof(int) * (size_t)ncols, stream());
      if (e == hipSuccess && !bad && !too_long) {
        hipLaunchKernelGGL(transp_slot_kernel, dim3(std::min((nrows + 3) / 4, 65536)), dim3(256), 0, stream(), nrows, ind, col,
                           T->ind, cursor, key);
        hipLaunchKernelGGL(transp_sort_kernel, dim3(std::min((ncols + 255) / 256, 65536)), dim3(256), 0, stream(), ncols, T->ind,
                           key);
// ... 231 lines not shown
```

### pysparse_amd/csrc/psp_internal.h

```cpp
#pragma once
#include <hip/hip_runtime.h>

#include <cstdarg>
#include <cstdint>
#include <cstdio>
#include <initializer_list>
#include <mutex>
#include <string>

#include "pysparse_hip.h"

namespace psp {

int fail(int code, const char *fmt, ...) __attribute__((format(printf, 2, 3)));
const char *tuning_env(const char *name);
void note_solve(const char *loop, int launches_per_iter, int vec_bytes_per_row, int dinv_streamed);
void note_fallback();
bool single_kernel_loops_enabled();
void setup_mark(const char *label);
struct HandleEntry {
  std::recursive_mutex mu;
  hipEvent_t ev = nullptr;
  hipStream_t last = nullptr;
  int ev_dev = -1;
// ... 301 lines not shown
  struct psp_mcsr *multi = nullptr;
  bool host = false;
};

namespace psp {
inline void op_lock_add(HandleLock &L, const psp_op *op) {
  if (!op || op->kind == 0) return;
  L.add(op);
  L.add(op->csr);
  L.add(op->sss);
  L.add(op->ssor);
  if (op->jac) {
    L.add(op->jac);
    L.add(op->jac->A.csr);
    L.add(op->jac->A.sss);
  }
}
inline void jacobi_lock_add(HandleLock &L, const psp_jacobi *K) {
  if (!K) return;
  L.add(K);
  L.add(K->A.csr);
  L.add(K->A.sss);
}
}
#define PSP_API_GUARD_OPS(A, K)      \
  psp::HandleLock psp_api_guard_;    \
  psp::op_lock_add(psp_api_guard_, A); \
  psp::op_lock_add(psp_api_guard_, K); \
  psp_api_guard_.lock()
#define PSP_API_GUARD_JAC(K)            \
  psp::HandleLock psp_api_guard_;       \
  psp::jacobi_lock_add(psp_api_guard_, K); \
  psp_api_guard_.lock()

namespace psp {
struct PcgDev {
  double rho, rho1, alpha, beta, normr, tolb, n2b, relres;
  int status;
  int info, iter, stag;
  int it;
  int maxit;
  int xpend;
  int stag0;
  int head_rho0;
  int head_beta0;
  int pend_maxit;
  double alpha_x;
};
struct MinresDev {
  double beta, beta_old, alpha, c, c_old, s, s_old, eta, norm_rmr, norm_r0, errtol, relres;
  double c1, c2;
  double r1, r2, r3, c_eta;
  int status;
  int stop;
  int skip;
  int info, iter, it_max;
};
struct KryDev {
  double r[32];
  int status;
  int code;
  int iter, maxit;
};
struct KryArg {
  const KryDev *S = nullptr;
  int i0 = 0, i1 = 0, i2 = 0;
};
int op_apply(const psp_op *op, const double *x_dev, double *y_dev);
inline psp_csr *op_native_csr(const psp_op *op) {
  if (!op) return nullptr;
  if (op->kind == PSP_OP_CSR) return op->csr;
  if (op->kind == PSP_OP_SSS) return op->sss->full;
  return nullptr;
}
int csr_spmv_launch(const psp_csr *A, const double *x, double *y, const double *dotv,
                    double *partials, int *nparts, const int *skip = nullptr);
int csr_spmv_pfused_launch(const psp_csr *A, const double *r, const double *dinv, const double *p_old,
                           double *p_new, double *q, double beta, bool first, double *partials, int *nparts,
                           const PcgDev *dstate, int *available);
int csr_spmv_pfx_launch(const psp_csr *A, const double *r, const double *dinv, const double *p_old, double *p_new,
                        double *q, double *x, double *partials, int *nparts, const PcgDev *dstate, int *available);
int csr_spmv_scaled_launch(const psp_csr *A, const double *x, double xdiv, double *y, double *partials,
                           int *nparts, int *available, const int *skip = nullptr,
                           const double *xdiv_dev = nullptr);
int csr_reordered_view(const psp_csr *A, psp_csr **R, const int **perm, const int **inv);
int reorder_gather(int n, const int *perm_dev, const double *x, double *xp, const int *skip);
bool csr_spmv_has_skip(const psp_csr *A);
int csr_spmv_overlap(const psp_csr *A, const double *x, double *y, const double *dotv,
                     double *partials, int *nparts, int row_a, int row_b, int (*wait)(void *),
                     void *ctx, const int *skip = nullptr);
int dinv_register(const double *v, long n);
void dinv_unregister(const double *v);
bool dinv_constant(const double *v, long n, double *c);
int jacobi_apply_dev(psp_jacobi *K, const double *x, double *y);
struct W4View {
  int no;
  int offs[12];
  int grid3[3];
  int constv;
  double cval[12];
  const double *valT;
  const unsigned short *mask;
  int stripe, grid;
};
int csr_w4_view(const psp_csr *A, W4View *out, int *available);
bool mid_applicable(const psp_csr *A, int n, const double *dinv);
int pcg_mid_loop(const psp_csr *A, const double *dinv, int n, double *x, double *r, double *p, double *q, double n2b,
                 double tolb, double normr0, double rho0, int maxit, int *info, int *iter, double *relres, double *hist);
bool brick_applicable(const psp_csr *A, int n);
int pcg_brick_loop(const psp_csr *A, const double *dinv, int n, double *x, double *r, double *p, double *q, double n2b,
                   double tolb, double normr0, double rho0, int maxit, int *info, int *iter, double *relres, double *hist);
bool brick_minres_applicable(const psp_csr *A, int n);
int minres_brick_loop(const psp_csr *A, const double *dinv, int n, double *x, double *v_hat, double *v_hat_old, double *y,
                      double *w, double *w_old, double *v, double *av, double norm_r0, double beta0, double errtol, int it_max,
                      int *info, int *iter, double *relres, double *hist);
bool mid_minres_applicable(const psp_csr *A, int n);
int minres_mid_loop(const psp_csr *A, const double *dinv, int n, double *x, double *v_hat, double *v_hat_old, double *y,
                    double *w, double *w_old, double *v, double *av, double norm_r0, double beta0, double errtol, int it_max,
                    int *info, int *iter, double *relres, double *hist);
constexpr int kCoopFallback = 1;
bool coop_applicable(const psp_csr *A, int n);
int pcg_coop_loop(const psp_csr *A, const double *dinv, int n, double *x, double *r, double *p, double *q, double n2b,
                  double tolb, double normr0, double rho0, int maxit, int *info, int *iter, double *relres,
                  double *hist);
int minres_coop_loop(const psp_csr *A, const double *dinv, int n, double *x, double *v_hat, double *v_hat_old,
                     double *y, double *w, double *w_old, double *v, double *av, double norm_r0, double beta0,
                     double errtol, int it_max, int *info, int *iter, double *relres, double *hist);
namespace cpu {
int csr_create(int nrows, int ncols, int nnz, const int *ind, const int *col, const double *val, psp_csr **out);
int csr_destroy(psp_csr *A);
int csr_poisson(int nx, int ny, int nz, psp_csr **out);
int csr_download(const psp_csr *A, int *ind, int *col, double *val);
int csr_diagonal(const psp_csr *A, double *diag);
int csr_matvec(const psp_csr *A, const double *x, ptrdiff_t incx, double *y, ptrdiff_t incy, bool transp);
int sss_create(int n, int nnz, const int *ind, const int *col, const double *val, const double *diag, psp_sss **out);
int sss_destroy(psp_sss *S);
int sss_poisson(int nx, int ny, int nz, psp_sss **out);
int sss_download(const psp_sss *S, int *ind, int *col, double *val, double *diag);
int sss_getitem(const psp_sss *S, int i, int j, double *value);
int sss_matvec(const psp_sss *S, const double *x, ptrdiff_t incx, double *y, ptrdiff_t incy);
int jacobi_create(int n, const double *diag, double omega, int steps, const psp_op *A, psp_jacobi **out);
int jacobi_destroy(psp_jacobi *K);
int jacobi_precon(const psp_jacobi *K, const double *x, double *y);
int pcg(const psp_op *A, const psp_op *K, int n, double *x, const double *b, double tol, int maxit, int *info,
        int *iter, double *relres, double *hist);
int minres(const psp_op *A, const psp_op *K, int n, double *x, const double *b, double tol, int maxit, int *info,
           int *iter, double *relres, double *hist);
}
bool placement_enabled();
bool placement_applies(const psp_csr *A, size_t n);
int place_operands(const psp_csr *A, size_t nx, size_t ny, int want_x, double **y_out, double **x_out, double *report);
int host_stage(const psp_csr *A, size_t nx, size_t ny, double **x, double **y);
void host_stage_trim();
int multi_destroy(psp_mcsr *M);
int multi_matvec_host(psp_mcsr *M, const double *x_host, ptrdiff_t incx, double *y_host, ptrdiff_t incy);
int multi_diagonal_host(psp_mcsr *M, double *diag_host);
int multi_jacobi_setup(psp_mcsr *M, double omega);
int multi_jacobi_apply_host(psp_mcsr *M, const double *x_host, double *y_host);
int multi_pcg(psp_mcsr *M, bool jacobi, int n, double *x_host, const double *b_host, double tol, int maxit,
              int *info, int *iter, double *relres, double *hist_host);
int multi_minres(psp_mcsr *M, bool jacobi, int n, double *x_host, const double *b_host, double tol, int maxit,
                 int *info, int *iter, double *relres, double *hist_host);
int multi_describe(const psp_mcsr *M, char *buf, int cap);
int ssor_apply_dev(psp_ssor *K, const double *b, double *x);
int ssor_error_check(psp_ssor *K);
int ssor_apply_host(psp_ssor *K, const double *b, double *x);
}
// ... 1 lines not shown
```

### pysparse_amd/csrc/psp_solvers.hip

```cpp
#include <algorithm>
#include <cmath>
#include <cstdlib>
#include <cstring>
#include <initializer_list>
#include <mutex>
#include <utility>
#include <vector>

#include "psp_internal.h"

using namespace psp;

namespace psp {
int k_dot(long n, const double *x, const double *y, double *partials, int *nparts);
int k_residual(long n, const double *b, double *r, const double *dinv, double *partials, int *nparts);
int k_pupdate(long n, const double *r, const double *dinv, double beta, bool first, double *p,
              const PcgDev *st = nullptr);
int k_px_update(long n, const double *r, const double *dinv, double *p, double *x, double *partials,
                int *nparts, const PcgDev *dstate, double beta = 0.0, double alpha = 0.0, bool first = false,
                bool xpend = false);
int k_x_update(long n, double alpha, const double *p, double *x, double *partials, int *nparts,
               const PcgDev *dstate);
int k_r_update(long n, double alpha, const double *q, const double *dinv, double *r, double *partials,
               int *nparts, const PcgDev *dstate);
// ... 208 lines not shown
}

}



__device__ __forceinline__ void pcg_finish(PcgDev *st, int code, int iter) {
  st->status = 1;
  st->info = code;
  st->iter = iter;
  st->relres = st->normr / st->n2b;
}

__device__ __forceinline__ void pcg_scalar_pq(PcgDev *st, const double *__restrict__ scal) {
  if (st->status) return;
  const double pq = scal[0];
  if (pq == 0.0) {
    pcg_finish(st, -6, st->it);
    return;
  }
  const double alpha = st->rho / pq;
  st->alpha = alpha;
  if (alpha == 0.0) st->stag = 1;
}

__device__ __forceinline__ void pcg_scalar_xr(PcgDev *st, const double *__restrict__ scal, double *__restrict__ hist) {
  if (st->status) return;
  const int it = st->it;
  if (st->stag == 0) st->stag = (scal[2] == 0.0) ? 1 : 0;
  const double normr = sqrt(scal[0]);
  st->normr = normr;
  if (hist) hist[it] = normr;
  if (normr <= st->tolb) {
    pcg_finish(st, 0, it);
  } else if (st->stag == 1) {
    pcg_finish(st, -5, it);
  } else if (it == st->maxit) {
    pcg_finish(st, -1, it + 1);
  } else {
    const double rho1 = st->rho, rho = scal[1];
    st->rho1 = rho1;
    st->rho = rho;
    st->it = it + 1;
    if (rho == 0.0) {
      pcg_finish(st, -2, it + 1);
    } else {
      const double beta = rho / rho1;
      if (beta == 0.0)
        pcg_finish(st, -6, it + 1);
      else
        st->beta = beta;
    }
  }
}

enum PcgScalarOp { kOpPq = 0, kOpXr = 1, kOpLazyX = 2, kOpLazyPq = 3, kOpLazyR = 4 };

template <int OP>
__global__ __launch_bounds__(kReduceBlock) void pcg_finish_scalar_kernel(const double *__restrict__ src, int count,
                                                                         int nvals, int stride, int raw,
                                                                         double *__restrict__ out, PcgDev *st,
                                                                         double *__restrict__ hist);
template <int OP>
static int pcg_reduce_then(const double *partials, int nparts, int nvals, double *out_dev, PcgDev *st,
                           double *hist_dev);

static int pcg_async_enabled() {
  static const int on = [] {
    const char *e = psp::tuning_env("PSP_PCG_ASYNC");
    return e ? atoi(e) : 1;
  }();
  return on;
}

static int pcg_graph_enabled() {
  static const int on = [] {
    const char *e = psp::tuning_env("PSP_PCG_GRAPH");
    return e ? atoi(e) : 0;
  }();
  return on;
}

static int pcg_enqueue_batch(psp_csr *Acsr, const double *dinv, int n, double *x, double *r, double **pp,
                             double **pp2, double *q, PcgDev *st, double *hist_dev, int batch) {
  Workspace *w;
  PSP_TRY(workspace(&w));
  int np;
  for (int i = 0; i < batch; ++i) {
    int fusedp = 0;
    PSP_TRY(csr_spmv_pfused_launch(Acsr, r, dinv, *pp, *pp2, q, 0.0, false, w->partials, &np, st, &fusedp));
    if (fusedp) {
      std::swap(*pp, *pp2);
    } else {
      PSP_TRY(k_pupdate(n, r, dinv, 0.0, false, *pp, st));
      PSP_TRY(csr_spmv_launch(Acsr, *pp, q, *pp, w->partials, &np, &st->status));
    }
    double *p = *pp;
    PSP_TRY(pcg_reduce_then<kOpPq>(w->partials, np, 1, w->scal_dev, st, nullptr));
    PSP_TRY(k_xr_update(n, 0.0, p, q, dinv, x, r, w->partials, &np, st));
    PSP_TRY(pcg_reduce_then<kOpXr>(w->partials, np, 3, w->scal_dev + 4, st, hist_dev));
  }
  PSP_LAUNCH_CHECK();
  return PSP_OK;
}

static int pcg_async_loop(psp_csr *Acsr, const double *dinv, int n, double *x, double *r, double *p,
                          double *p2, double *q, double n2b, double tolb, double normr0, double rho0, int maxit,
                          int *info, int *iter, double *relres, double *hist) {
  constexpr int kBatch = 16;
  PcgDev *st = nullptr;
  PcgDev *hst = nullptr;
  double *hist_dev = nullptr;
  hipStream_t own = nullptr, prev = nullptr;
  bool swapped = false;
  hipGraph_t graph = nullptr;
  hipGraphExec_t exec = nullptr;
  int enqueued = 0;
  static_assert(sizeof(PcgDev) <= kStateBytes, "state slab");
  Workspace *wst;
  PSP_TRY(workspace(&wst));
  st = static_cast<PcgDev *>(wst->state_dev);
  hst = static_cast<PcgDev *>(wst->state_host);
  hipError_t e = hipSuccess;
  if (hist) e = hipMalloc((void **)&hist_dev, sizeof(double) * ((size_t)maxit + 1));
  if (e != hipSuccess) {
    return fail(PSP_ENOMEM, "pcg: state allocation failed: %s", hipGetErrorString(e));
  }
  int rc = PSP_OK;
#define PCG_TRY(call)            \
  do {                           \
    rc = (call);                 \
    if (rc != PSP_OK) goto done; \
  } while (0)
#define PCG_HIP(call)                                                \
  do {                                                               \
    hipError_t e_ = (call);                                          \
    if (e_ != hipSuccess) {                                          \
      rc = fail(PSP_ENODEV, "%s: %s", #call, hipGetErrorString(e_)); \
      goto done;                                                     \
    }                                                                \
  } while (0)
  if (hist_dev) PCG_HIP(hipMemsetAsync(hist_dev, 0xff, sizeof(double) * ((size_t)maxit + 1), stream()));
  memset(hst, 0, sizeof(PcgDev));
  hst->rho = rho0;
  hst->rho1 = 1.0;
  hst->normr = normr0;
  hst->tolb = tolb;
  hst->n2b = n2b;
  hst->it = 1;
  hst->maxit = maxit;
  PCG_HIP(hipMemcpyAsync(st, hst, sizeof(PcgDev), hipMemcpyHostToDevice, stream()));
  enqueued = std::min(kBatch, maxit);
  PCG_TRY(pcg_enqueue_batch(Acsr, dinv, n, x, r, &p, &p2, q, st, hist_dev, enqueued));
  PCG_HIP(hipMemcpyAsync(hst, st, sizeof(PcgDev), hipMemcpyDeviceToHost, stream()));
  PCG_HIP(hipStreamSynchronize(stream()));
  if (!hst->status) {
    bool use_graph = pcg_graph_enabled() != 0;
    if (use_graph) {
      if (hipStreamCreateWithFlags(&own, hipStreamNonBlocking) == hipSuccess) {
        prev = swap_stream(own);
        swapped = true;
        if (hipStreamBeginCapture(own, hipStreamCaptureModeThreadLocal) == hipSuccess) {
          const int brc = pcg_enqueue_batch(Acsr, dinv, n, x, r, &p, &p2, q, st, hist_dev, kBatch);
          const hipError_t ce = hipStreamEndCapture(own, &graph);
          if (brc != PSP_OK || ce != hipSuccess || graph == nullptr ||
              hipGraphInstantiate(&exec, graph, nullptr, nullptr, 0) != hipSuccess) {
            exec = nullptr;
          }
        }
        if (exec == nullptr) {
          (void)hipGetLastError();
          swap_stream(prev);
          swapped = false;
        }
      }
      use_graph = exec != nullptr;
    }
    while (!hst->status) {
      if (use_graph) {
        PCG_HIP(hipGraphLaunch(exec, stream()));
      } else {
        const int batch = std::max(1, std::min(kBatch, maxit - enqueued));
        PCG_TRY(pcg_enqueue_batch(Acsr, dinv, n, x, r, &p, &p2, q, st, hist_dev, batch));
        enqueued += batch;
      }
      PCG_HIP(hipMemcpyAsync(hst, st, sizeof(PcgDev), hipMemcpyDeviceToHost, stream()));
      PCG_HIP(hipStreamSynchronize(stream()));
    }
  }
  *info = hst->info;
  *iter = hst->iter;
  *relres = hst->relres;
  if (hist) {
    const int cnt = std::min(hst->iter, maxit);
    if (cnt >= 1)
      PCG_HIP(hipMemcpy(hist + 1, hist_dev + 1, sizeof(double) * (size_t)cnt, hipMemcpyDeviceToHost));
  }
done:
#undef PCG_TRY
#undef PCG_HIP
  if (swapped) {
    (void)hipStreamSynchronize(own);
    swap_stream(prev);
  }
  if (exec) (void)hipGraphExecDestroy(exec);
  if (graph) (void)hipGraphDestroy(graph);
  if (own) (void)hipStreamDestroy(own);
  if (hist_dev) (void)hipFree(hist_dev);
  return rc;
}


__device__ __forceinline__ void pcg_lazy_scalar_x(PcgDev *st, const double *__restrict__ scal) {
  if (st->status) return;
  if (st->xpend) {
    const int stag = st->stag0 || scal[0] == 0.0;
    st->xpend = 0;
    if (stag) {
      st->stag = 1;
      pcg_finish(st, -5, st->it - 1);
      return;
    }
  }
  if (st->head_rho0) {
    pcg_finish(st, -2, st->it);
    return;
  }
  if (st->head_beta0) pcg_finish(st, -6, st->it);
}

__device__ __forceinline__ void pcg_lazy_scalar_pq(PcgDev *st, const double *__restrict__ scal) {
  if (st->status) return;
  const double pq = scal[0];
  if (pq == 0.0) {
    pcg_finish(st, -6, st->it);
    return;
  }
  const double alpha = st->rho / pq;
  st->alpha = alpha;
  st->alpha_x = alpha;
  st->stag0 = alpha == 0.0 ? 1 : 0;
  st->xpend = 1;
}

__device__ __forceinline__ void pcg_lazy_scalar_r(PcgDev *st, const double *__restrict__ scal, double *__restrict__ hist) {
  if (st->status) return;
  const int it = st->it;
  const double normr = sqrt(scal[0]);
  st->normr = normr;
  if (hist) hist[it] = normr;
  if (normr <= st->tolb) {
    pcg_finish(st, 0, it);
  } else if (it == st->maxit) {
    st->pend_maxit = 1;
    st->status = 1;
  } else {
    const double rho1 = st->rho, rho = scal[1];
    st->rho1 = rho1;
    st->rho = rho;
    st->it = it + 1;
    st->head_rho0 = rho == 0.0 ? 1 : 0;
    st->head_beta0 = 0;
    if (rho != 0.0) {
      const double beta = rho / rho1;
      st->beta = beta;
      st->head_beta0 = beta == 0.0 ? 1 : 0;
    }
  }
}

template <int OP>
__global__ __launch_bounds__(kReduceBlock) void pcg_finish_scalar_kernel(const double *__restrict__ src, int count,
                                                                         int nvals, int stride, int raw,
                                                                         double *__restrict__ out, PcgDev *st,
                                                                         double *__restrict__ hist) {
  if (st->status) return;
  __shared__ double sh[kOneBlockGroups];
  reduce_block(src, count, nvals, stride, raw != 0, out, sh);
  if (threadIdx.x == 0) {
    if constexpr (OP == kOpPq) pcg_scalar_pq(st, out);
    if constexpr (OP == kOpXr) pcg_scalar_xr(st, out, hist);
    if constexpr (OP == kOpLazyX) pcg_lazy_scalar_x(st, out);
    if constexpr (OP == kOpLazyPq) pcg_lazy_scalar_pq(st, out);
    if constexpr (OP == kOpLazyR) pcg_lazy_scalar_r(st, out, hist);
  }
}

__global__ __launch_bounds__(kReduceBlock) void pcg_finish_xpq_kernel(const double *__restrict__ src_x, int count_x,
                                                                      int stride_x, int raw_x,
                                                                      const double *__restrict__ src_q, int count_q,
                                                                      int stride_q, int raw_q, double *__restrict__ out_x,
                                                                      double *__restrict__ out_q, PcgDev *st) {
  if (st->status) return;
  __shared__ double sh[kOneBlockGroups];
  reduce_block(src_x, count_x, 1, stride_x, raw_x != 0, out_x, sh);
  reduce_block(src_q, count_q, 1, stride_q, raw_q != 0, out_q, sh);
  if (threadIdx.x == 0) {
    pcg_lazy_scalar_x(st, out_x);
    pcg_lazy_scalar_pq(st, out_q);
  }
}

template <int OP>
static int pcg_reduce_then(const double *partials, int nparts, int nvals, double *out_dev, PcgDev *st,
                           double *hist_dev) {
  const double *src;
  int count, stride;
  bool raw;
  PSP_TRY(fold_stage(partials, nparts, nvals, &src, &count, &stride, &raw));
  hipLaunchKernelGGL((pcg_finish_scalar_kernel<OP>), dim3(1), dim3(kReduceBlock), 0, stream(), src, count, nvals,
                     stride, raw ? 1 : 0, out_dev, st, hist_dev);
  PSP_LAUNCH_CHECK();
  return PSP_OK;
}

static int pcg_reduce_xpq(Workspace *w, const double *parts_x, int np_x, const double *parts_q, int np_q, double *out_x,
                          double *out_q, PcgDev *st) {
  const double *const parts[2] = {parts_x, parts_q};
  const int np[2] = {np_x, np_q}, fslot[2] = {2, 0};
  const double *src[2];
  int count[2], stride[2];
  bool raw[2];
  (void)w;
  PSP_TRY(fold_stage2(parts, np, fslot, src, count, stride, raw));
  hipLaunchKernelGGL(pcg_finish_xpq_kernel, dim3(1), dim3(kReduceBlock), 0, stream(), src[0], count[0], stride[0],
                     raw[0] ? 1 : 0, src[1], count[1], stride[1], raw[1] ? 1 : 0, out_x, out_q, st);
  PSP_LAUNCH_CHECK();
  return PSP_OK;
}

static int pcg_lazy_enabled() {
  const char *e = psp::tuning_env("PSP_PCG_LAZYX");
  return e ? atoi(e) : 1;
}

static int pcg_lazypf_mode(int n) {
  const char *e = psp::tuning_env("PSP_PCG_LAZYPF");
  return e ? atoi(e) : (n >= (1 << 21) ? 1 : 0);
}

static int pcg_async_loop_lazy(psp_csr *Acsr, const double *dinv, int n, double *x, double *r, double *p, double *p2,
                               double *q, double n2b, double tolb, double normr0, double rho0, int maxit,
                               int *info, int *iter, double *relres, double *hist) {
  constexpr int kBatch = 16;
  double *const P[2] = {p, p2};
  int usepf = (p2 && pcg_lazypf_mode(n)) ? 1 : 0;
  Workspace *w;
  PSP_TRY(workspace(&w));
  PcgDev *st = nullptr, *hst = nullptr;
  double *hist_dev = nullptr;
  static_assert(sizeof(PcgDev) <= kStateBytes, "state slab");
  Workspace *wst;
  PSP_TRY(workspace(&wst));
  st = static_cast<PcgDev *>(wst->state_dev);
  hst = static_cast<PcgDev *>(wst->state_host);
  hipError_t e = hipSuccess;
  if (hist) e = hipMalloc((void **)&hist_dev, sizeof(double) * ((size_t)maxit + 1));
  if (e != hipSuccess) {
    return fail(PSP_ENOMEM, "pcg: state allocation failed: %s", hipGetErrorString(e));
  }
  int rc = PSP_OK;
  int enqueued = 0, np = 0;
  double *stag_parts = w->partials + 2 * (size_t)kMaxParts;
  const bool merge_xpq = [] {
    const char *e = psp::tuning_env("PSP_PCG_MERGE_XPQ");
    return e ? atoi(e) != 0 : true;
  }();
#define PCG_TRY(call)            \
  do {                           \
    rc = (call);                 \
    if (rc != PSP_OK) goto done; \
  } while (0)
#define PCG_HIP(call)                                                \
  do {                                                               \
    hipError_t e_ = (call);                                          \
    if (e_ != hipSuccess) {                                          \
      rc = fail(PSP_ENODEV, "%s: %s", #call, hipGetErrorString(e_)); \
      goto done;                                                     \
    }                                                                \
  } while (0)
  if (hist_dev) PCG_HIP(hipMemsetAsync(hist_dev, 0xff, sizeof(double) * ((size_t)maxit + 1), stream()));
  memset(hst, 0, sizeof(PcgDev));
  hst->rho = rho0;
  hst->rho1 = 1.0;
  hst->normr = normr0;
  hst->tolb = tolb;
  hst->n2b = n2b;
  hst->it = 1;
  hst->maxit = maxit;
  PCG_HIP(hipMemcpyAsync(st, hst, sizeof(PcgDev), hipMemcpyHostToDevice, stream()));
  do {
    const int batch = std::max(1, std::min(kBatch, maxit - enqueued));
    for (int i = 0; i < batch; ++i) {
      int np_x = 0;
      if (usepf) {
        const int e = enqueued + i + 1;
        int av = 0;
        PCG_TRY(csr_spmv_pfx_launch(Acsr, r, dinv, P[(e - 1) & 1], P[e & 1], q, x, w->partials, &np, st, &av));
        if (av) {
          PCG_TRY(pcg_reduce_xpq(w, stag_parts, np, w->partials, np, w->scal_dev + 8, w->scal_dev, st));
          PCG_TRY(k_r_update(n, 0.0, q, dinv, r, w->partials, &np, st));
          PCG_TRY(pcg_reduce_then<kOpLazyR>(w->partials, np, 2, w->scal_dev + 4, st, hist_dev));
          continue;
        }
        usepf = 0;
      }
      PCG_TRY(k_px_update(n, r, dinv, p, x, w->partials, &np_x, st));
      if (!merge_xpq) PCG_TRY(pcg_reduce_then<kOpLazyX>(stag_parts, np_x, 1, w->scal_dev + 8, st, nullptr));
      PCG_TRY(csr_spmv_launch(Acsr, p, q, p, w->partials, &np, &st->status));
      if (merge_xpq)
        PCG_TRY(pcg_reduce_xpq(w, stag_parts, np_x, w->partials, np, w->scal_dev + 8, w->scal_dev, st));
      else
        PCG_TRY(pcg_reduce_then<kOpLazyPq>(w->partials, np, 1, w->scal_dev, st, nullptr));
      PCG_TRY(k_r_update(n, 0.0, q, dinv, r, w->partials, &np, st));
      PCG_TRY(pcg_reduce_then<kOpLazyR>(w->partials, np, 2, w->scal_dev + 4, st, hist_dev));
    }
    PCG_HIP(hipGetLastError());
    enqueued += batch;
    PCG_HIP(hipMemcpyAsync(hst, st, sizeof(PcgDev), hipMemcpyDeviceToHost, stream()));
    PCG_HIP(hipStreamSynchronize(stream()));
  } while (!hst->status);
  if (usepf) p = P[hst->it & 1];
  if (hst->xpend) {
    double s[1];
    PCG_TRY(k_x_update(n, hst->alpha_x, p, x, w->partials, &np, nullptr));
    PCG_TRY(finish_partials(stag_parts, np, 1, w->scal_dev + 8));
    PCG_TRY(fetch_scalars(w->scal_dev + 8, 1, s));
    if (hst->pend_maxit) {
      const bool stag = hst->stag0 || s[0] == 0.0;
      hst->info = stag ? -5 : -1;
      hst->iter = stag ? maxit : maxit + 1;
      hst->relres = hst->normr / hst->n2b;
    }
  }
  *info = hst->info;
  *iter = hst->iter;
  *relres = hst->relres;
  if (hist) {
    const int cnt = std::min(hst->iter, maxit);
    if (cnt >= 1)
      PCG_HIP(hipMemcpy(hist + 1, hist_dev + 1, sizeof(double) * (size_t)cnt, hipMemcpyDeviceToHost));
  }
done:
#undef PCG_TRY
#undef PCG_HIP
  if (hist_dev) (void)hipFree(hist_dev);
  return rc;
}

static bool norm2_unsafe(double sq) { return !(sq >= 1e-280 && sq <= 1e280); }
static int abs_max(int n, const double *v, double *out);
static int robust_nrm2(Workspace *w, int n, const double *v, double sq, double *out) {
  if (!norm2_unsafe(sq)) {
    *out = sqrt(sq);
    return PSP_OK;
  }
  double vmax = 0.0;
  PSP_TRY(abs_max(n, v, &vmax));
  if (vmax == 0.0 || vmax != vmax || std::isinf(vmax)) {
    *out = vmax == 0.0 ? 0.0 : sqrt(sq);
    return PSP_OK;
  }
  int e = 0;
  (void)frexp(vmax, &e);
  DevVecs mem;
  double *t;
  PSP_TRY(mem.alloc(n, &t));
  PSP_HIP(hipMemcpyAsync(t, v, sizeof(double) * (size_t)n, hipMemcpyDeviceToDevice, stream()));
  PSP_TRY(k_scal(n, ldexp(1.0, -e), t));
  int np;
  double s1;
  PSP_TRY(k_dot(n, t, t, w->partials, &np));
  PSP_TRY(reduce_fetch(w, np, 1, &s1));
  *out = ldexp(sqrt(s1), e);
  return PSP_OK;
}

static int pcg_device_core(const psp_op *A, const psp_op *K, psp_csr *Acsr_forced, const double *dinv_forced,
                           int n, double *x, const double *b, double tol, int maxit, int *info, int *iter,
                           double *relres, double *hist) {
  note_solve("pcg_no_iterations", 0, 0, 0);
  Workspace *w;
  PSP_TRY(workspace(&w));
  DevVecs mem;
  double *r, *p, *q, *z = nullptr;
  psp_csr *Acsr = Acsr_forced ? Acsr_forced : op_native_csr(A);
  const double *dinv = Acsr_forced ? dinv_forced : fused_dinv(K);
  const bool fused = Acsr != nullptr && (Acsr_forced || K == nullptr || dinv != nullptr);
  double *p2 = nullptr;
  PSP_TRY(mem.alloc(n, &r));
  if (fused) {
    PSP_TRY(mem.alloc_operands(Acsr, n, &q, &p, &p2));
  } else {
    PSP_TRY(mem.alloc(n, &p));
    PSP_TRY(mem.alloc(n, &q));
    if (K) PSP_TRY(mem.alloc(n, &z));
  }

  double s[4];
  int np;

  PSP_TRY(k_dot(n, b, b, w->partials, &np));
  PSP_TRY(reduce_fetch(w, np, 1, s));
  double n2b;
  PSP_TRY(robust_nrm2(w, n, b, s[0], &n2b));
  if (n2b == 0.0) {
    PSP_HIP(hipMemsetAsync(x, 0, sizeof(double) * (size_t)n, stream()));
    PSP_HIP(hipStreamSynchronize(stream()));
    *info = 0;
    *relres = 0.0;
    *iter = 0;
    return PSP_OK;
  }

  *info = -1;
  const double tolb = tol * n2b;

  if (Acsr_forced)
    PSP_TRY(csr_spmv_launch(Acsr, x, r, nullptr, nullptr, nullptr));
  else
    PSP_TRY(op_apply(A, x, r));
  PSP_TRY(k_residual(n, b, r, fused ? dinv : nullptr, w->partials, &np));
  PSP_TRY(reduce_fetch(w, np, 2, s));
  double normr;
  PSP_TRY(robust_nrm2(w, n, r, s[0], &normr));
  double rho_next = s[1];
  if (hist) hist[0] = normr;

  if (normr <= tolb) {
    *info = 0;
    *relres = normr / n2b;
    *iter = 0;
    return PSP_OK;
  }

  const bool sk = single_kernel_loops_enabled();
  double dcst;
  const int dstream = (dinv && !dinv_constant(dinv, n, &dcst)) ? 1 : 0;
  if (sk && fused && maxit >= 1 && rho_next != 0.0 && mid_applicable(Acsr, n, dinv)) {
    const int rc = pcg_mid_loop(Acsr, dinv, n, x, r, p, q, n2b, tolb, normr, rho_next, maxit, info, iter, relres, hist);
    if (rc != kCoopFallback) {
      note_solve("pcg_mid", 1, 0, dstream);
      return rc;
    }
    note_fallback();
  }
  if (sk && fused && maxit >= 1 && rho_next != 0.0 && brick_applicable(Acsr, n)) {
    const int rc = pcg_brick_loop(Acsr, dinv, n, x, r, p, q, n2b, tolb, normr, rho_next, maxit, info, iter, relres, hist);
    if (rc != kCoopFallback) {
      note_solve("pcg_brick", 1, 0, dstream);
      return rc;
    }
    note_fallback();
  }
  if (sk && fused && maxit >= 1 && coop_applicable(Acsr, n)) {
    const int rc = pcg_coop_loop(Acsr, dinv, n, x, r, p, q, n2b, tolb, normr, rho_next, maxit, info, iter, relres, hist);
    if (rc != kCoopFallback) {
      note_solve("pcg_coop", 1, 0, dstream);
      return rc;
    }
    note_fallback();
  }
  if (fused && maxit >= 1 && pcg_async_enabled() && csr_spmv_has_skip(Acsr)) {
    if (rho_next == 0.0) {
      *info = -2;
      *iter = 1;
      *relres = normr / n2b;
      return PSP_OK;
    }
    const int lazy_mode = pcg_lazy_enabled();
    const int rl = n > (1 << 21) ? 2 : 0;
    if ((lazy_mode == 2 || (lazy_mode == 1 && (n < (1 << 24) || n >= 3 * (1 << 23)))) && !pcg_graph_enabled()) {
      const bool pf = p2 && pcg_lazypf_mode(n);
      note_solve(pf ? "pcg_lazy_pf" : "pcg_lazy", (pf ? 4 : 5) + rl, (pf ? 56 : 64) + 16 * dstream, dstream);
      return pcg_async_loop_lazy(Acsr, dinv, n, x, r, p, p2, q, n2b, tolb, normr, rho_next, maxit, info, iter,
                                 relres, hist);
    }
    note_solve("pcg_eager", 6 + rl, 72 + 16 * dstream, dstream);
    return pcg_async_loop(Acsr, dinv, n, x, r, p, p2, q, n2b, tolb, normr, rho_next, maxit, info, iter,
                          relres, hist);
  }
  note_solve("pcg_host_scalars", -1, -1, dstream);

  double rho = 1.0, rho1, beta = 0.0, alpha, pq;
  int stag = 0;
  int it;
  for (it = 1; it <= maxit; ++it) {
    const double *zsrc = r;
    const double *zdinv = dinv;
    if (!fused) {
      zdinv = nullptr;
      if (K) {
        PSP_TRY(op_apply(K, r, z));
        zsrc = z;
      }
      PSP_TRY(k_dot(n, r, zsrc, w->partials, &np));
      PSP_TRY(reduce_fetch(w, np, 1, s));
      rho_next = s[0];
    }
    rho1 = rho;
    rho = rho_next;
    if (rho == 0.0) {
      *info = -2;
      break;
    }
    if (it > 1) {
      beta = rho / rho1;
      if (beta == 0.0) {
        *info = -6;
        break;
      }
    }
    int fusedp = 0;
    if (fused)
      PSP_TRY(csr_spmv_pfused_launch(Acsr, r, dinv, p, p2, q, beta, it == 1, w->partials, &np, nullptr, &fusedp));
    if (fusedp) {
      std::swap(p, p2);
    } else {
      PSP_TRY(k_pupdate(n, zsrc, zdinv, it == 1 ? 0.0 : beta, it == 1, p));
    }

    if (fusedp) {
    } else if (Acsr) {
      PSP_TRY(csr_spmv_launch(Acsr, p, q, p, w->partials, &np));
    } else {
      PSP_TRY(op_apply(A, p, q));
      PSP_TRY(k_dot(n, p, q, w->partials, &np));
    }
    PSP_TRY(reduce_fetch(w, np, 1, s));
    pq = s[0];
    if (pq == 0.0) {
      *info = -6;
      break;
    }
    alpha = rho / pq;
    if (alpha == 0.0) stag = 1;

    PSP_TRY(k_xr_update(n, alpha, p, q, fused ? dinv : nullptr, x, r, w->partials, &np));
    PSP_TRY(reduce_fetch(w, np, 3, s));
    if (stag == 0) stag = (s[2] == 0.0);
    normr = sqrt(s[0]);
    rho_next = s[1];
    if (hist) hist[it] = normr;

    if (normr <= tolb) {
      *info = 0;
      break;
    }
    if (stag == 1) {
      *info = -5;
      break;
    }
  }
  *iter = it;
  *relres = normr / n2b;
  PSP_HIP(hipStreamSynchronize(stream()));
  return PSP_OK;
}


struct PermutedSystem {
  psp_csr *R = nullptr;
  const int *perm = nullptr, *inv = nullptr;
// ... 77 lines not shown
  if (beta < 0.0) {
    st->status = 1;
    st->skip = 1;
    st->info = -3;
    return;
  }
  beta = sqrt(beta);
  st->beta = beta;
  const double c_oold = st->c_old;
  const double c_old = st->c;
  const double s_oold = st->s_old;
  const double s_old = st->s;
  st->c_old = c_old;
  st->s_old = s_old;
  const double r1_hat = c_old * alpha - c_oold * s_old * beta_old;
  const double r1 = sqrt(r1_hat * r1_hat + beta * beta);
  const double r2 = s_old * alpha + c_oold * c_old * beta_old;
  const double r3 = s_oold * beta_old;
  if (r1 == 0.0) {
    st->status = 1;
    st->skip = 1;
    st->info = -6;
    return;
  }
  const double c = r1_hat / r1;
  const double s_ = beta / r1;
  st->c = c;
  st->s = s_;
  st->r1 = r1;
  st->r2 = r2;
  st->r3 = r3;
  st->c_eta = c * st->eta;
  st->eta = -s_ * st->eta;
  const double norm_rmr = st->norm_rmr * fabs(s_);
  st->norm_rmr = norm_rmr;
  if (hist) hist[st->iter] = norm_rmr;
  const bool conv = norm_rmr < st->errtol * st->norm_r0;
  if (st->iter >= st->it_max || conv) {
    st->stop = 1;
    st->skip = 1;
    st->relres = norm_rmr / st->norm_r0;
    st->info = conv ? 0 : -1;
  } else {
    st->iter += 1;
  }
}

template <int OP>
__global__ __launch_bounds__(kReduceBlock) void minres_finish_scalar_kernel(const double *__restrict__ src, int count,
                                                                            int stride, int raw, double *__restrict__ out,
                                                                            MinresDev *st, double *__restrict__ hist) {
  if (st->status) return;
  __shared__ double sh[kOneBlockGroups];
  reduce_block(src, count, 1, stride, raw != 0, out, sh);
  if (threadIdx.x == 0) {
    if constexpr (OP == kMrAlpha) minres_scalar_alpha(st, out);
    if constexpr (OP == kMrBeta) minres_scalar_beta(st, out, hist);
  }
}

template <int OP>
static int minres_reduce_then(const double *partials, int nparts, double *out_dev, MinresDev *st, double *hist_dev) {
  const double *src;
  int count, stride;
  bool raw;
  PSP_TRY(fold_stage(partials, nparts, 1, &src, &count, &stride, &raw));
  hipLaunchKernelGGL((minres_finish_scalar_kernel<OP>), dim3(1), dim3(kReduceBlock), 0, stream(), src, count, stride,
                     raw ? 1 : 0, out_dev, st, hist_dev);
  PSP_LAUNCH_CHECK();
  return PSP_OK;
}

static int minres_async_enabled() {
  static const int on = [] {
    const char *e = psp::tuning_env("PSP_MINRES_ASYNC");
    return e ? atoi(e) : 1;
  }();
  return on;
}

static int minres_async_loop(psp_csr *Acsr, const double *dinv, bool hasK, int n, double *x, double *v_hat,
                             double *v_hat_old, double *y, double *y2, double *wv, double *w_old, double *v,
                             double *av, double norm_r0, double beta0, double errtol, int it_max, int *info,
                             int *iter, double *relres, double *hist) {
  constexpr int kBatch = 16;
  Workspace *w;
  PSP_TRY(workspace(&w));
  MinresDev *st = nullptr, *hst = nullptr;
  double *hist_dev = nullptr;
  static_assert(sizeof(MinresDev) <= kStateBytes, "state slab");
  st = static_cast<MinresDev *>(w->state_dev);
  hst = static_cast<MinresDev *>(w->state_host);
  hipError_t e = hipSuccess;
  if (hist) e = hipMalloc((void **)&hist_dev, sizeof(double) * ((size_t)it_max + 1));
  if (e != hipSuccess) {
    return fail(PSP_ENOMEM, "minres: state allocation failed: %s", hipGetErrorString(e));
  }
  if (hist_dev) (void)hipMemsetAsync(hist_dev, 0xff, sizeof(double) * ((size_t)it_max + 1), stream());
  int rc = PSP_OK;
  int enqueued = 0, np = 0;
#define MR_TRY(call)             \
  do {                           \
    rc = (call);                 \
    if (rc != PSP_OK) goto done; \
  } while (0)
#define MR_HIP(call)                                                 \
  do {                                                               \
    hipError_t e_ = (call);                                          \
    if (e_ != hipSuccess) {                                          \
      rc = fail(PSP_ENODEV, "%s: %s", #call, hipGetErrorString(e_)); \
      goto done;                                                     \
    }                                                                \
  } while (0)
  bool v_ready = false;
  const bool wx_vnext = [] {
    const char *e = psp::tuning_env("PSP_MINRES_WXV");
    return e ? atoi(e) != 0 : true;
  }();
  memset(hst, 0, sizeof(MinresDev));
  hst->beta = beta0;
  hst->beta_old = 1.0;
  hst->c = 1.0;
  hst->c_old = 1.0;
  hst->s = 0.0;
  hst->s_old = 0.0;
  hst->eta = beta0;
  hst->norm_rmr = norm_r0;
  hst->norm_r0 = norm_r0;
  hst->errtol = errtol;
  hst->iter = 1;
  hst->it_max = it_max;
  hst->info = -1;
  MR_HIP(hipMemcpyAsync(st, hst, sizeof(MinresDev), hipMemcpyHostToDevice, stream()));
  do {
    const int batch = std::max(1, std::min(kBatch, it_max - enqueued));
    for (int i = 0; i < batch; ++i) {
      const double *vsrc = hasK ? y : v_hat;
      int scaled = 0;
      if (!hasK || y2)
        MR_TRY(csr_spmv_scaled_launch(Acsr, vsrc, 1.0, av, w->partials, &np, &scaled, &st->skip, &st->beta));
      if (!scaled) {
        if (!v_ready) MR_TRY(k_scale_div(n, vsrc, 1.0, v, st));
        MR_TRY(csr_spmv_launch(Acsr, v, av, v, w->partials, &np, &st->skip));
      }
      MR_TRY(minres_reduce_then<kMrAlpha>(w->partials, np, w->scal_dev, st, nullptr));
      double *ynew = (scaled && hasK) ? y2 : y;
      MR_TRY(k_lanczos(n, av, 0.0, 0.0, v_hat, v_hat_old, dinv, ynew, w->partials, &np, st));
      std::swap(v_hat, v_hat_old);
      if (scaled && hasK) std::swap(y, y2);
      MR_TRY(minres_reduce_then<kMrBeta>(w->partials, np, w->scal_dev + 4, st, hist_dev));
      if (!scaled && wx_vnext) {
        MR_TRY(k_minres_wx_vnext(n, v, hasK ? y : v_hat, wv, w_old, x, st));
        v_ready = true;
      } else {
        MR_TRY(k_minres_wx(n, scaled ? vsrc : v, 0.0, 0.0, 0.0, 0.0, wv, w_old, x, scaled != 0, 1.0, st));
      }
      std::swap(wv, w_old);
    }
    MR_HIP(hipGetLastError());
    enqueued += batch;
    MR_HIP(hipMemcpyAsync(hst, st, sizeof(MinresDev), hipMemcpyDeviceToHost, stream()));
    MR_HIP(hipStreamSynchronize(stream()));
  } while (!hst->status && !hst->stop);
  *info = hst->info;
  *iter = hst->iter;
  if (hst->info == 0 || hst->info == -1) *relres = hst->relres;
  if (hist) {
    const int cnt = std::min(hst->iter, it_max) - ((hst->info == -3 || hst->info == -6) ? 1 : 0);
    if (cnt >= 1)
      MR_HIP(hipMemcpy(hist + 1, hist_dev + 1, sizeof(double) * (size_t)cnt, hipMemcpyDeviceToHost));
  }
done:
#undef MR_TRY
#undef MR_HIP
  if (hist_dev) (void)hipFree(hist_dev);
  return rc;
}

static int minres_device_core(const psp_op *A, const psp_op *K, psp_csr *Acsr_forced, const double *dinv_forced,
                              int n, double *x, const double *b, double errtol, int it_max, int *info, int *iter,
                              double *relres, double *hist) {
  note_solve("minres_no_iterations", 0, 0, 0);
  Workspace *w;
  PSP_TRY(workspace(&w));
  DevVecs mem;
  double *v_hat_old = nullptr, *v_hat = nullptr, *y = nullptr, *wv, *w_old, *v, *av = nullptr;
  const bool hasK = Acsr_forced ? dinv_forced != nullptr : K != nullptr;
  psp_csr *Acsr = Acsr_forced ? Acsr_forced : op_native_csr(A);
  const double *dinv = Acsr_forced ? dinv_forced : fused_dinv(K);
  const bool kfused = Acsr_forced || (K == nullptr) || dinv != nullptr;
  double *y2 = nullptr;
  if (Acsr && kfused && placement_applies(Acsr, n)) {
    double *xa, *xb;
    PSP_TRY(mem.alloc_operands(Acsr, n, &av, &xa, &xb));
    if (hasK) {
      y = xa;
      y2 = xb;
    } else {
      v_hat = xa;
      v_hat_old = xb;
    }
  }
  if (!v_hat_old) PSP_TRY(mem.alloc(n, &v_hat_old));
  if (!v_hat) PSP_TRY(mem.alloc(n, &v_hat));
  PSP_TRY(mem.alloc(n, &wv));
  PSP_TRY(mem.alloc(n, &w_old));
  PSP_TRY(mem.alloc(n, &v));
  if (!av) PSP_TRY(mem.alloc(n, &av));
  if (hasK && !y) PSP_TRY(mem.alloc(n, &y));
  if (hasK && kfused && Acsr && !y2) PSP_TRY(mem.alloc(n, &y2));
  const size_t bytes = sizeof(double) * (size_t)n;
  double s[4];
  int np;

  *iter = 0;
  PSP_HIP(hipMemsetAsync(v_hat_old, 0, bytes, stream()));
  if (Acsr_forced)
    PSP_TRY(csr_spmv_launch(Acsr, x, v_hat, nullptr, nullptr, nullptr));
  else
    PSP_TRY(op_apply(A, x, v_hat));
  PSP_TRY(k_residual(n, b, v_hat, kfused ? dinv : nullptr, w->partials, &np));
  PSP_TRY(reduce_fetch(w, np, 2, s));
  double norm_r0_;
  PSP_TRY(robust_nrm2(w, n, v_hat, s[0], &norm_r0_));
  const double norm_r0 = norm_r0_;
  double beta = s[1];
  if (hasK) {
    if (Acsr_forced)
      PSP_TRY(k_jacobi_first(n, v_hat, dinv, y));
    else
      PSP_TRY(op_apply(K, v_hat, y));
    if (!kfused) {
      PSP_TRY(k_dot(n, v_hat, y, w->partials, &np));
      PSP_TRY(reduce_fetch(w, np, 1, s));
      beta = s[0];
    }
  }
  if (beta < 0.0) {
    *info = -3;
    PSP_HIP(hipStreamSynchronize(stream()));
    return PSP_OK;
  }
  beta = sqrt(beta);
  double beta_old = 1.0;
  double c = 1.0, c_old = 1.0, s_ = 0.0, s_old = 0.0, c_oold, s_oold;
  PSP_HIP(hipMemsetAsync(wv, 0, bytes, stream()));
  PSP_HIP(hipMemsetAsync(w_old, 0, bytes, stream()));
  double eta = beta;
  double norm_rmr = norm_r0;
  if (hist) hist[0] = norm_rmr;

  const bool sk = single_kernel_loops_enabled();
  double dcst;
  const int dstream = (hasK && dinv && !dinv_constant(dinv, n, &dcst)) ? 1 : 0;
  if (sk && Acsr && kfused && it_max >= 1 && !(norm_rmr < errtol * norm_r0) && (!hasK || dinv) && mid_minres_applicable(Acsr, n)) {
    const int rc = minres_mid_loop(Acsr, hasK ? dinv : nullptr, n, x, v_hat, v_hat_old, y, wv, w_old, v, av, norm_r0,
                                   beta, errtol, it_max, info, iter, relres, hist);
    if (rc != kCoopFallback) {
      note_solve("minres_mid", 1, 0, dstream);
      return rc;
    }
    note_fallback();
  }
  if (sk && Acsr && kfused && it_max >= 1 && !(norm_rmr < errtol * norm_r0) && (!hasK || dinv) && brick_minres_applicable(Acsr, n)) {
    const int rc = minres_brick_loop(Acsr, hasK ? dinv : nullptr, n, x, v_hat, v_hat_old, y, wv, w_old, v, av, norm_r0,
                                     beta, errtol, it_max, info, iter, relres, hist);
    if (rc != kCoopFallback) {
      note_solve("minres_brick", 1, 0, dstream);
      return rc;
    }
    note_fallback();
  }
  if (sk && Acsr && kfused && it_max >= 1 && !(norm_rmr < errtol * norm_r0) && coop_applicable(Acsr, n)) {
    const int rc = minres_coop_loop(Acsr, hasK ? dinv : nullptr, n, x, v_hat, v_hat_old, y, wv, w_old, v, av, norm_r0,
                                    beta, errtol, it_max, info, iter, relres, hist);
    if (rc != kCoopFallback) {
      note_solve("minres_coop", 1, 0, dstream);
      return rc;
    }
    note_fallback();
  }
  if (Acsr && kfused && minres_async_enabled() && it_max >= 1 && !(norm_rmr < errtol * norm_r0)) {
    note_solve("minres_async", 5 + (n > (1 << 21) ? 2 : 0), 88 + 8 * dstream, dstream);
    return minres_async_loop(Acsr, dinv, hasK, n, x, v_hat, v_hat_old, y, y2, wv, w_old, v, av, norm_r0,
                             beta, errtol, it_max, info, iter, relres, hist);
  }
  note_solve("minres_host_scalars", -1, -1, dstream);

  while (true) {
    if (*iter >= it_max || norm_rmr < errtol * norm_r0) break;
    *iter += 1;

    const double *vsrc = hasK ? y : v_hat;
    const double vdiv = beta;
    int scaled = 0;
    if (Acsr && kfused && (!hasK || y2))
      PSP_TRY(csr_spmv_scaled_launch(Acsr, vsrc, vdiv, av, w->partials, &np, &scaled));
    if (!scaled) PSP_TRY(k_scale_div(n, vsrc, beta, v));
    if (scaled) {
    } else if (Acsr) {
      PSP_TRY(csr_spmv_launch(Acsr, v, av, v, w->partials, &np));
    } else {
      PSP_TRY(op_apply(A, v, av));
      PSP_TRY(k_dot(n, v, av, w->partials, &np));
    }
    PSP_TRY(reduce_fetch(w, np, 1, s));
    const double alpha = s[0];
    const double dconst1 = alpha / beta, dconst2 = beta / beta_old;
    if (kfused) {
      double *ynew = (scaled && hasK) ? y2 : y;
      PSP_TRY(k_lanczos(n, av, dconst1, dconst2, v_hat, v_hat_old, dinv, ynew, w->partials, &np));
      std::swap(v_hat, v_hat_old);
      if (scaled && hasK) std::swap(y, y2);
    } else {
      PSP_TRY(k_lanczos_plain(n, av, dconst1, dconst2, v_hat, v_hat_old));
      std::swap(v_hat, v_hat_old);
      PSP_TRY(op_apply(K, v_hat, y));
      PSP_TRY(k_dot(n, v_hat, y, w->partials, &np));
    }
    PSP_TRY(reduce_fetch(w, np, 1, s));
    beta_old = beta;
    beta = s[0];
    if (beta < 0.0) {
      *info = -3;
      PSP_HIP(hipStreamSynchronize(stream()));
      return PSP_OK;
    }
    beta = sqrt(beta);

    c_oold = c_old;
    c_old = c;
    s_oold = s_old;
    s_old = s_;
    const double r1_hat = c_old * alpha - c_oold * s_old * beta_old;
    const double r1 = sqrt(r1_hat * r1_hat + beta * beta);
    const double r2 = s_old * alpha + c_oold * c_old * beta_old;
    const double r3 = s_oold * beta_old;
    if (r1 == 0.0) {
      *info = -6;
      PSP_HIP(hipStreamSynchronize(stream()));
      return PSP_OK;
    }
    c = r1_hat / r1;
    s_ = beta / r1;

    PSP_TRY(k_minres_wx(n, scaled ? vsrc : v, r1, r2, r3, c * eta, wv, w_old, x, scaled != 0, vdiv));
    std::swap(wv, w_old);
    eta = -s_ * eta;
    norm_rmr *= fabs(s_);
    if (hist) hist[*iter] = norm_rmr;
  }

  *relres = norm_rmr / norm_r0;
  *info = (norm_rmr < errtol * norm_r0) ? 0 : -1;
  PSP_HIP(hipStreamSynchronize(stream()));
  return PSP_OK;
}

static int minres_permuted(const psp_op *A, const psp_op *K, int n, double *x, const double *b, double errtol,
                           int it_max, int *info, int *iter, double *relres, double *hist) {
  DevVecs mem;
  PermutedSystem ps;
  int active = 0;
  if (minres_async_enabled()) PSP_TRY(ps.enter(A, K, n, mem, x, b, &active));
  if (!active)
    return minres_device_core(A, K, nullptr, nullptr, n, x, b, errtol, it_max, info, iter, relres, hist);
  const int rc =
      minres_device_core(A, K, ps.R, ps.dp, n, ps.xp, ps.bp, errtol, it_max, info, iter, relres, hist);
// ... 1525 lines not shown
```

### pysparse_amd/device.py

```python
import ctypes as C

import numpy as np

from . import _capi
from ._capi import check, lib


def _f64(a, n, what):
    if not isinstance(a, np.ndarray) or a.ndim != 1 or a.dtype != np.float64 or a.shape[0] != n:
        raise ValueError("%s must be a 1-dimensional double array of appropriate size." % what)
    return a


def _ptr(a):
    return a.ctypes.data_as(C.c_void_p)


class DeviceBuffer:

    def __init__(self, n, dtype=np.float64):
        self.n = int(n)
        self.dtype = np.dtype(dtype)
        self.nbytes = self.n * self.dtype.itemsize
        p = C.c_void_p()
# ... 104 lines not shown
        h = C.c_void_p()
        check(lib().psp_csr_create_multi(shape[0], shape[1], val.shape[0], _ptr(ind), _ptr(col), _ptr(val),
                                         _ptr(dv), len(dv), C.byref(h)))
        return cls(h)

    def multi_info(self):
        a, b, c = C.c_int(), C.c_int(), C.c_int()
        check(lib().psp_csr_multi_info(self._h, C.byref(a), C.byref(b), C.byref(c)))
        return a.value, b.value, bool(c.value)

    @classmethod
    def poisson_big(cls, nx, ny, nz=0):
        h = C.c_void_p()
        check(lib().psp_csr_poisson_big(nx, ny, nz, C.byref(h)))
        A = cls(h)
        A.nnz = int(lib().psp_csr_nnz64(h))
        return A

    @classmethod
    def poisson_big_slab(cls, nx, ny, nz, row_lo, row_hi, col_shift, ncols_local):
        h = C.c_void_p()
        check(lib().psp_csr_poisson_big_slab(nx, ny, nz, row_lo, row_hi, col_shift, ncols_local, C.byref(h)))
        A = cls(h)
        A.nnz = int(lib().psp_csr_nnz64(h))
        return A

    @classmethod
    def poisson_slab(cls, nx, ny, nz, row_lo, row_hi, col_shift, ncols_local):
        h = C.c_void_p()
        check(lib().psp_csr_poisson_slab(nx, ny, nz, row_lo, row_hi, col_shift, ncols_local, C.byref(h)))
        return cls(h)

    def matvec(self, x, y):
        _f64(x, self.shape[1], "arg 1")
        _f64(y, self.shape[0], "arg 2")
        es = x.itemsize
        check(lib().psp_csr_matvec_stride(self._h, _ptr(x), x.strides[0] // es, _ptr(y), y.strides[0] // es))

    def matvec_transp(self, x, y):
        _f64(x, self.shape[0], "arg 1")
        _f64(y, self.shape[1], "arg 2")
        es = x.itemsize
        check(lib().psp_csr_matvec_transp_stride(self._h, _ptr(x), x.strides[0] // es, _ptr(y),
                                                 y.strides[0] // es))

    def matvec_dev(self, x_ptr, y_ptr):
        check(lib().psp_csr_matvec_dev(self._h, x_ptr, y_ptr))

    def download(self):
        ind = np.empty(self.shape[0] + 1, dtype=np.int32)
        col = np.empty(self.nnz, dtype=np.int32)
        val = np.empty(self.nnz, dtype=np.float64)
        check(lib().psp_csr_download(self._h, _ptr(ind), _ptr(col), _ptr(val)))
        return ind, col, val

    def diagonal(self):
        d = np.empty(self.shape[0])
        check(lib().psp_csr_diagonal(self._h, _ptr(d)))
        return d

    def set_variant(self, v):
        check(lib().psp_csr_set_variant(self._h, int(v)))

    def set_schedule(self, strip_rows):
        check(lib().psp_csr_set_schedule(self._h, int(strip_rows)))

    def kernel_info(self):
        name = C.create_string_buffer(160)
        info = (C.c_int * 4)()
        check(lib().psp_csr_kernel_info(self._h, name, 160, info))
        return name.value.decode(), {"nb": info[0], "max_blocks": info[1], "scheduled": bool(info[2]),
                                     "half_band": info[3], "setup_ms": self.setup_info()["reorder_ms"]}

    def release_arrays(self):
        check(lib().psp_csr_release_arrays(self._h))

    def prepare(self, expected_products):
        check(lib().psp_csr_prepare(self._h, int(expected_products)))

    def setup_info(self):
        v = (C.c_double * 4)()
        check(lib().psp_csr_setup_info(self._h, v))
        return {"reorder_ms": v[0], "products_counted": int(v[1]), "reorder_after": int(v[2]), "reorder_state": int(v[3])}

    def renumbering(self):
        perm = np.empty(self.shape[0], dtype=np.int32)
        have = C.c_int()
        check(lib().psp_csr_renumbering(self._h, perm.ctypes.data, C.byref(have)))
        self.renumbered_on = {0: None, 1: "host", 2: "device"}[have.value]
        return perm if have.value else None

    @property
    def device_bytes(self):
        return lib().psp_csr_device_bytes(self._h)

    def close(self):
        if getattr(self, "_h", None):
            lib().psp_csr_destroy(self._h)
            self._h = None

    def __del__(self):
        try:
            self.close()
        except Exception:
            pass


class DeviceSSS:

    def __init__(self, handle):
        self._h = handle
        n, nz = C.c_int(), C.c_int()
        check(lib().psp_sss_shape(handle, C.byref(n), C.byref(nz)))
        self.n = n.value
        self.shape = (self.n, self.n)
        self.nnz = nz.value

    @classmethod
    def from_arrays(cls, n, ind, col, val, diag):
        ind = np.ascontiguousarray(ind, dtype=np.int32)
        col = np.ascontiguousarray(col, dtype=np.int32)
        val = np.ascontiguousarray(val, dtype=np.float64)
        diag = np.ascontiguousarray(diag, dtype=np.float64)
        h = C.c_void_p()
        check(lib().psp_sss_create(n, val.shape[0], _ptr(ind), _ptr(col), _ptr(val), _ptr(diag), C.byref(h)))
        return cls(h)

    @classmethod
    def poisson(cls, nx, ny, nz=0):
        h = C.c_void_p()
        check(lib().psp_sss_poisson(nx, ny, nz, C.byref(h)))
        return cls(h)

    def matvec(self, x, y):
        _f64(x, self.n, "arg 1")
        _f64(y, self.n, "arg 2")
        es = x.itemsize
        check(lib().psp_sss_matvec_stride(self._h, _ptr(x), x.strides[0] // es, _ptr(y), y.strides[0] // es))

    matvec_transp = matvec

    def matvec_dev(self, x_ptr, y_ptr):
        check(lib().psp_sss_matvec_dev(self._h, x_ptr, y_ptr))

    def set_variant(self, v):
        check(lib().psp_sss_set_variant(self._h, int(v)))

    def prepare(self, expected_products):
        check(lib().psp_sss_prepare(self._h, int(expected_products)))

    def setup_info(self):
        v = (C.c_double * 4)()
        check(lib().psp_sss_setup_info(self._h, v))
        return {"reorder_ms": v[0], "products_counted": int(v[1]), "reorder_after": int(v[2]), "reorder_state": int(v[3])}

    def kernel_info(self):
        name = C.create_string_buffer(64)
        info = (C.c_int * 4)()
        check(lib().psp_sss_kernel_info(self._h, name, 64, info))
        return name.value.decode(), {"nb": info[0], "max_blocks": info[1], "scheduled": bool(info[2]),
                                     "half_band": info[3], "setup_ms": self.setup_info()["reorder_ms"]}

    def __getitem__(self, ij):
        if not (isinstance(ij, tuple) and len(ij) == 2 and all(isinstance(t, (int, np.integer)) for t in ij)):
            raise IndexError("slices not supported")
        i, j = int(ij[0]), int(ij[1])
# ... 263 lines not shown
```

Baseline: 6143.

## Detect symmetric CSR diagonal layout and run PCG/MINRES SpMV through half-storage SSS kernel

Adds a device check that verifies whether a CSR matrix stored in the diagonal (w4) layout is exactly symmetric. When it is, the code builds lower-triangle value, diagonal and mask tables and routes SpMV inside the async PCG and MINRES loops through the SSS half-storage kernel. This roughly halves the off-diagonal value bytes read per product. The cost is a one-time check and table build, extra device memory, and skipping the fused p-update path when symmetric tables are used.

```diff
diff --git a/include/pysparse_hip.h b/include/pysparse_hip.h
--- a/include/pysparse_hip.h
+++ b/include/pysparse_hip.h
@@ -107,6 +107,7 @@
 int psp_csr_prepare(psp_csr_t *A, long long expected_products);
 int psp_csr_release_arrays(psp_csr_t *A);
 int psp_csr_setup_info(psp_csr_t *A, double *info4);
+int psp_csr_sym_info(psp_csr_t *A, double *info4);
 int psp_csr_renumbering(psp_csr_t *A, int *perm_host, int *available);
 int64_t psp_csr_device_bytes(const psp_csr_t *A);
 
diff --git a/pysparse_amd/_capi.py b/pysparse_amd/_capi.py
--- a/pysparse_amd/_capi.py
+++ b/pysparse_amd/_capi.py
@@ -11,7 +11,7 @@
 psp_csr_create psp_csr_poisson psp_csr_poisson_slab psp_csr_poisson_big psp_csr_poisson_big_slab psp_csr_nnz64 psp_csr_create64 psp_csr_random_banded psp_csr_download_rows psp_csr_destroy psp_csr_shape
 psp_csr_download psp_csr_diagonal psp_csr_matvec psp_csr_matvec_stride psp_csr_matvec_transp
 psp_csr_matvec_transp_stride psp_csr_matvec_dev psp_csr_matvec_transp_dev psp_csr_set_variant
-psp_csr_set_schedule psp_csr_kernel_info psp_csr_prepare psp_csr_setup_info psp_csr_release_arrays psp_csr_renumbering psp_csr_device_bytes
+psp_csr_set_schedule psp_csr_kernel_info psp_csr_prepare psp_csr_setup_info psp_csr_sym_info psp_csr_release_arrays psp_csr_renumbering psp_csr_device_bytes
 psp_csr_poisson_multi psp_csr_create_multi psp_csr_multi_info psp_csr_multi_spmv_time psp_csr_multi_phase_time psp_multi_plan
 psp_sss_create psp_sss_poisson psp_sss_destroy psp_sss_shape psp_sss_download psp_sss_getitem
 psp_sss_matvec psp_sss_matvec_stride psp_sss_matvec_dev psp_sss_device_bytes
@@ -153,6 +153,7 @@
         "psp_last_solve_info": [C.c_char_p, i, C.POINTER(i)], "psp_set_single_kernel_loops": [i],
         "psp_csr_release_arrays": [vp], "psp_csr_prepare": [vp, C.c_longlong], "psp_sss_prepare": [vp, C.c_longlong],
         "psp_csr_setup_info": [vp, C.POINTER(d)], "psp_sss_setup_info": [vp, C.POINTER(d)],
+        "psp_csr_sym_info": [vp, C.POINTER(d)],
     }
     for name, argtypes in sig.items():
         f = getattr(L, name)
diff --git a/pysparse_amd/csrc/psp_csr_abi.h b/pysparse_amd/csrc/psp_csr_abi.h
--- a/pysparse_amd/csrc/psp_csr_abi.h
+++ b/pysparse_amd/csrc/psp_csr_abi.h
@@ -337,6 +337,9 @@
       if (it->second.dia_mask32) (void)hipFree(it->second.dia_mask32);
       if (it->second.dia_mask64) (void)hipFree(it->second.dia_mask64);
       if (it->second.dia_offs_dev) (void)hipFree(it->second.dia_offs_dev);
+      if (it->second.sym_valL) (void)hipFree(it->second.sym_valL);
+      if (it->second.sym_diag) (void)hipFree(it->second.sym_diag);
+      if (it->second.sym_mask) (void)hipFree(it->second.sym_mask);
       g_extra.erase(it);
     }
   }
@@ -599,6 +602,23 @@
   info4[1] = (double)it->second.products;
   info4[2] = (double)reorder_after();
   info4[3] = (double)it->second.reorder_state;
+  return PSP_OK;
+}
+
+int psp_csr_sym_info(psp_csr_t *A, double *info4) {
+  PSP_API_GUARD_H(A);
+  if (!A || !info4) return fail(PSP_EINVAL, "psp_csr_sym_info: NULL argument");
+  info4[0] = 0.0;
+  info4[1] = -1.0;
+  info4[2] = info4[3] = 0.0;
+  psp::CsrExtra *ex;
+  PSP_TRY(ensure_sym_state(A, &ex));
+  if (!ex) return PSP_OK;
+  std::lock_guard<std::mutex> lk(g_sym_mu);
+  info4[0] = (double)ex->sym_state;
+  info4[1] = (double)ex->sym_tab;
+  info4[2] = ex->sym_ms;
+  info4[3] = (double)ex->sym_fallbacks;
   return PSP_OK;
 }
 
diff --git a/pysparse_amd/csrc/psp_csr_kernels.h b/pysparse_amd/csrc/psp_csr_kernels.h
--- a/pysparse_amd/csrc/psp_csr_kernels.h
+++ b/pysparse_amd/csrc/psp_csr_kernels.h
@@ -1361,12 +1361,59 @@
   }
 }
 
+struct SymMirror {
+  int k[16];
+};
+
+__global__ void w4_sym_check_kernel(int n, int no, DiaOffs offs, SymMirror mirror, int dslot,
+                                    const double *__restrict__ valT, const unsigned short *__restrict__ mask,
+                                    int *__restrict__ bad) {
+  int found = 0;
+  for (long r = (long)blockIdx.x * blockDim.x + threadIdx.x; r < n; r += (long)gridDim.x * blockDim.x) {
+    const unsigned m = mask[r];
+    if (!((m >> dslot) & 1u)) found = 1;
+    const double *vp = valT + (size_t)(r / kDiaRows) * no * kDiaRows + (size_t)(r % kDiaRows);
+    for (int k = 0; k < no; ++k) {
+      if (k == dslot || !((m >> k) & 1u)) continue;
+      const long c = r + offs.o[k];
+      const int km = mirror.k[k];
+      if (c < 0 || c >= n || km < 0) {
+        found = 1;
+        continue;
+      }
+      const double *vc = valT + (size_t)(c / kDiaRows) * no * kDiaRows + (size_t)(c % kDiaRows);
+      if (!((mask[c] >> km) & 1u) ||
+          __double_as_longlong(vp[(size_t)k * kDiaRows]) != __double_as_longlong(vc[(size_t)km * kDiaRows]))
+        found = 1;
+    }
+  }
+  if (found) atomicOr(bad, 1);
+}
+
+__global__ void w4_sym_tables_kernel(int n, int nol, const double *__restrict__ valT,
+                                     const unsigned short *__restrict__ mask, double *__restrict__ valL,
+                                     double *__restrict__ diag, unsigned short *__restrict__ smask) {
+  const int no = 2 * nol + 1;
+  for (long r = (long)blockIdx.x * blockDim.x + threadIdx.x; r < n; r += (long)gridDim.x * blockDim.x) {
+    const size_t blk = (size_t)(r / kDiaRows), i = (size_t)(r % kDiaRows);
+    const double *vp = valT + blk * no * kDiaRows + i;
+    double *lp = valL + blk * nol * kDiaRows + i;
+    for (int j = 0; j < nol; ++j) lp[(size_t)j * kDiaRows] = vp[(size_t)j * kDiaRows];
+    diag[r] = vp[(size_t)nol * kDiaRows];
+    const unsigned m = mask[r];
+    unsigned s = m & ((1u << nol) - 1u);
+    for (int j = 0; j < nol; ++j)
+      if ((m >> (no - 1 - j)) & 1u) s |= 1u << (8 + j);
+    smask[r] = (unsigned short)s;
+  }
+}
+
 template <int NOL, int FLAGS = 0>
 __global__ __launch_bounds__(256) void sss_spmv_w4(
     int n, int stripe, SssOffs offs, const double *__restrict__ valL, const double *__restrict__ diag,
     const unsigned short *__restrict__ mask, const double *__restrict__ x, double *__restrict__ y,
     const double *__restrict__ dotv, double *__restrict__ partials, const int *__restrict__ skip,
-    int use_div, double xdiv, const double *__restrict__ xdiv_dev, int dot_is_x) {
+    int use_div, double xdiv, const double *__restrict__ xdiv_dev, int dot_is_x, int pstripe) {
   if (skip && *skip) return;
   if (xdiv_dev) xdiv = *xdiv_dev;
   __shared__ double red[4];
@@ -1531,7 +1578,16 @@
     dsum = wave_sum(dsum);
     if (lane == 0) red[wid] = dsum;
     __syncthreads();
-    if (threadIdx.x == 0) partials[blockIdx.x] = red[0] + red[1] + red[2] + red[3];
+    if (threadIdx.x == 0) {
+      int slot = (int)blockIdx.x;
+      if (pstripe == 0) {
+        slot = vb;
+      } else if (pstripe > 0) {
+        const int q = vb / pstripe;
+        slot = (((q >> 3) * pstripe + vb % pstripe) << 3) + (q & 7);
+      }
+      partials[slot] = red[0] + red[1] + red[2] + red[3];
+    }
   }
 }
 
diff --git a/pysparse_amd/csrc/psp_csr_select.h b/pysparse_amd/csrc/psp_csr_select.h
--- a/pysparse_amd/csrc/psp_csr_select.h
+++ b/pysparse_amd/csrc/psp_csr_select.h
@@ -200,8 +200,60 @@
   return PSP_OK;
 }
 
+static int sym_product_enabled() {
+  const char *e = psp::tuning_env("PSP_SYM_PRODUCT");
+  return e ? atoi(e) != 0 : 1;
+}
+
+int csr_sym_product_ready(const psp_csr *A, int *ready) {
+  *ready = 0;
+  if (!sym_product_enabled() || A->variant >= 0) return PSP_OK;
+  psp::CsrExtra *ex;
+  PSP_TRY(ensure_sym_state(A, &ex));
+  if (!ex || ex->sym_state != 1) return PSP_OK;
+  PSP_TRY(ensure_sym_tables(A, ex));
+  if (ex->sym_tab != 1) {
+    std::lock_guard<std::mutex> lk(g_sym_mu);
+    ex->sym_fallbacks += 1;
+    return PSP_OK;
+  }
+  *ready = 1;
+  return PSP_OK;
+}
+
+int csr_spmv_sym_launch(const psp_csr *A, const double *x, double *y, const double *dotv, double *partials,
+                        int *nparts, const int *skip, int use_div, double xdiv, const double *xdiv_dev) {
+  psp::CsrExtra *ex;
+  {
+    std::lock_guard<std::mutex> lk(g_extra_mu);
+    ex = &g_extra[A];
+  }
+  if (ex->sym_tab != 1) return fail(PSP_EINVAL, "csr_spmv_sym_launch: the handle has no symmetric tables");
+  Variant v = decode_variant(A->variant);
+  if (A->w4_only) v.w4 = true;
+  const int sw = w4_stripe(A, v);
+  const int nblk = (A->nrows + kDiaRows - 1) / kDiaRows;
+  const int grid = w4_grid(nblk, sw);
+  int ss = spmv_stripe() >= 0 ? sw : 32;
+  if (ss <= 0 || grid % (8 * ss) != 0) ss = sw;
+  double *pbuf = partials;
+  if (partials && grid > kMaxParts) {
+    PSP_TRY(ensure_big_partials(ex, grid));
+    pbuf = ex->big_partials;
+  }
+  PSP_TRY(launch_sss_w4(sym_view(A, ex), ss, x, y, dotv, pbuf, skip, grid, use_div, xdiv, xdiv_dev, sw));
+  int np = grid;
+  if (pbuf != partials) {
+    np = kFold;
+    hipLaunchKernelGGL(fold_partials_kernel, dim3(np / 16), dim3(256), 0, stream(), pbuf, grid, partials, np);
+    PSP_LAUNCH_CHECK();
+  }
+  if (nparts) *nparts = np;
+  return PSP_OK;
+}
+
 int csr_spmv_scaled_launch(const psp_csr *A, const double *x, double xdiv, double *y, double *partials,
-                           int *nparts, int *available, const int *skip, const double *xdiv_dev) {
+                           int *nparts, int *available, const int *skip, const double *xdiv_dev, int sym) {
   *available = 0;
   static const bool on = [] {
     const char *e = psp::tuning_env("PSP_MINRES_SCALED");
@@ -210,6 +262,11 @@
   Variant v = decode_variant(A->variant);
   if (A->w4_only) v.w4 = true;
   if (!on || !v.w4 || A->nparts || A->nrows != A->ncols || A->nrows < 2) return PSP_OK;
+  if (sym) {
+    PSP_TRY(csr_spmv_sym_launch(A, x, y, x, partials, nparts, skip, 1, xdiv, xdiv_dev));
+    *available = 1;
+    return PSP_OK;
+  }
   const int stripe = w4_stripe(A, v);
   const int nblk = (A->nrows + kDiaRows - 1) / kDiaRows;
   const int grid = w4_grid(nblk, stripe);
@@ -234,7 +291,7 @@
     pbuf = ex->big_partials;
   }
   if (sss)
-    PSP_TRY(launch_sss_w4(A->sym_owner, stripe, x, y, x, pbuf, skip, grid, 1, xdiv, xdiv_dev));
+    PSP_TRY(launch_sss_w4(sss_view(A->sym_owner), stripe, x, y, x, pbuf, skip, grid, 1, xdiv, xdiv_dev));
   else
     PSP_TRY(launch_w4(A, ex, stripe, 0, nblk, x, y, x, pbuf, skip, grid, 1, xdiv, xdiv_dev));
   int np = grid;
@@ -580,7 +637,7 @@
         PSP_TRY(ensure_big_partials(ex, grid));
         pbuf = ex->big_partials;
       }
-      PSP_TRY(launch_sss_w4(S, stripe, x, y, dotv, pbuf, skip, grid));
+      PSP_TRY(launch_sss_w4(sss_view(S), stripe, x, y, dotv, pbuf, skip, grid));
       int np = grid;
       if (pbuf != partials) {
         np = kFold;
diff --git a/pysparse_amd/csrc/psp_csr_tables.h b/pysparse_amd/csrc/psp_csr_tables.h
--- a/pysparse_amd/csrc/psp_csr_tables.h
+++ b/pysparse_amd/csrc/psp_csr_tables.h
@@ -61,6 +61,15 @@
   int grid_nx = 0, grid_ny = 0;
   int constv_state = -1;
   double constv[16] = {0};
+  int sym_state = -1;
+  int sym_tab = -1;
+  int sym_nol = 0;
+  SssOffs sym_offs;
+  double *sym_valL = nullptr;
+  double *sym_diag = nullptr;
+  unsigned short *sym_mask = nullptr;
+  double sym_ms = 0.0;
+  long sym_fallbacks = 0;
 };
 
 }
@@ -618,37 +627,138 @@
   return PSP_OK;
 }
 
-static int launch_sss_w4(const psp_sss *S, int stripe, const double *x, double *y, const double *dotv,
+struct SssTables {
+  int n = 0, nol = 0;
+  SssOffs offs;
+  const double *valL = nullptr, *diag = nullptr;
+  const unsigned short *mask = nullptr;
+  bool soa = false;
+  int flags = 0;
+};
+
+static SssTables sss_view(const psp_sss *S) {
+  SssTables t;
+  t.n = S->n;
+  t.nol = S->w4_nol;
+  for (int i = 0; i < 8; ++i) t.offs.o[i] = S->w4_offs[i];
+  t.valL = S->w4_val;
+  t.diag = S->diag;
+  t.mask = S->w4_mask;
+  t.soa = S->w4_soa;
+  t.flags = (S->full->variant >= 0 ? S->full->variant : 0) >> 23 & 3;
+  return t;
+}
+
+static SssTables sym_view(const psp_csr *A, const psp::CsrExtra *ex) {
+  SssTables t;
+  t.n = A->nrows;
+  t.nol = ex->sym_nol;
+  t.offs = ex->sym_offs;
+  t.valL = ex->sym_valL;
+  t.diag = ex->sym_diag;
+  t.mask = ex->sym_mask;
+  return t;
+}
+
+static int launch_sss_w4(const SssTables &T, int stripe, const double *x, double *y, const double *dotv,
                          double *pbuf, const int *skip, int grid, int use_div = 0, double xdiv = 1.0,
-                         const double *xdiv_dev = nullptr) {
-  SssOffs so;
-  for (int i = 0; i < 8; ++i) so.o[i] = S->w4_offs[i];
-  const int flags = (S->full->variant >= 0 ? S->full->variant : 0) >> 23 & 3;
+                         const double *xdiv_dev = nullptr, int pstripe = -1) {
+  const int flags = T.flags;
 #define PSP_SW4_F(NOL, F)                                                                            \
-  hipLaunchKernelGGL((sss_spmv_w4<NOL, F>), dim3(grid), dim3(256), 0, stream(), S->n, stripe, so,     \
-                     S->w4_val, S->diag, S->w4_mask, x, y, dotv, pbuf, skip, use_div, xdiv, xdiv_dev,         \
-                     (dotv == x && !w4_dot_reload()) ? 1 : 0)
+  hipLaunchKernelGGL((sss_spmv_w4<NOL, F>), dim3(grid), dim3(256), 0, stream(), T.n, stripe, T.offs, \
+                     T.valL, T.diag, T.mask, x, y, dotv, pbuf, skip, use_div, xdiv, xdiv_dev,                 \
+                     (dotv == x && !w4_dot_reload()) ? 1 : 0, pstripe)
   static const bool shfl = [] {
     const char *e = psp::tuning_env("PSP_SSS_SHFL");
     return e ? atoi(e) != 0 : true;
   }();
 #define PSP_SW4(NOL)                                                                                 \
   case NOL:                                                                                          \
-    if (S->w4_soa) PSP_SW4_F(NOL, 12);                                                               \
+    if (T.soa) PSP_SW4_F(NOL, 12);                                                                   \
     else if (flags == 0 && shfl) PSP_SW4_F(NOL, 4);                                                  \
     else if (flags == 0) PSP_SW4_F(NOL, 0);                                                          \
     else if (flags == 1) PSP_SW4_F(NOL, 1);                                                          \
     else if (flags == 2) PSP_SW4_F(NOL, 2);                                                          \
     else PSP_SW4_F(NOL, 3);                                                                          \
     break
-  switch (S->w4_nol) {
+  switch (T.nol) {
     PSP_SW4(1); PSP_SW4(2); PSP_SW4(3); PSP_SW4(4); PSP_SW4(5); PSP_SW4(6); PSP_SW4(7); PSP_SW4(8);
     default:
-      return fail(PSP_EINVAL, "sss_spmv_w4: %d offsets", S->w4_nol);
+      return fail(PSP_EINVAL, "sss_spmv_w4: %d offsets", T.nol);
   }
 #undef PSP_SW4
 #undef PSP_SW4_F
   PSP_LAUNCH_CHECK();
+  return PSP_OK;
+}
+
+static std::mutex g_sym_mu;
+static int ensure_sym_state(const psp_csr *A, psp::CsrExtra **out) {
+  *out = nullptr;
+  if (A->nparts || A->multi || A->host || A->sym_owner || A->nrows != A->ncols || A->nrows < 2) return PSP_OK;
+  Variant v = decode_variant(A->variant);
+  if (A->w4_only) v.w4 = true;
+  if (!v.w4) return PSP_OK;
+  psp::CsrExtra *ex;
+  PSP_TRY(ensure_w4(A, &ex));
+  *out = ex;
+  std::lock_guard<std::mutex> lk(g_sym_mu);
+  if (ex->sym_state >= 0) return PSP_OK;
+  ex->sym_state = 0;
+  if (ex->dia_state != 1 || ex->dia_no > 16 || !ex->dia_mask || (ex->dia_no & 1) == 0) return PSP_OK;
+  const int no = ex->dia_no, nol = no / 2;
+  if (nol < 1 || nol > 8 || ex->dia_offs.o[nol] != 0) return PSP_OK;
+  SymMirror mir;
+  for (int k = 0; k < 16; ++k) mir.k[k] = -1;
+  for (int k = 0; k < no; ++k) {
+    if (ex->dia_offs.o[no - 1 - k] != -ex->dia_offs.o[k]) return PSP_OK;
+    mir.k[k] = no - 1 - k;
+  }
+  ScratchDev bad_mem;
+  PSP_HIP(hipMalloc(&bad_mem.p, sizeof(int)));
+  int *bad = (int *)bad_mem.p;
+  PSP_HIP(hipMemsetAsync(bad, 0, sizeof(int), stream()));
+  hipLaunchKernelGGL(w4_sym_check_kernel, dim3(std::min((A->nrows + 255) / 256, 16384)), dim3(256), 0, stream(),
+                     A->nrows, no, ex->dia_offs, mir, nol, ex->dia_val, ex->dia_mask, bad);
+  PSP_LAUNCH_CHECK();
+  int hbad = 1;
+  PSP_HIP(hipMemcpyAsync(&hbad, bad, sizeof(int), hipMemcpyDeviceToHost, stream()));
+  PSP_HIP(hipStreamSynchronize(stream()));
+  if (hbad == 0) ex->sym_state = 1;
+  return PSP_OK;
+}
+
+static int ensure_sym_tables(const psp_csr *A, psp::CsrExtra *ex) {
+  std::lock_guard<std::mutex> lk(g_sym_mu);
+  if (ex->sym_tab >= 0 || ex->sym_state != 1) return PSP_OK;
+  const auto t0 = std::chrono::steady_clock::now();
+  ex->sym_tab = 0;
+  const int n = A->nrows, nol = ex->dia_no / 2;
+  const size_t nblk = ((size_t)n + kDiaRows - 1) / kDiaRows;
+  const size_t nval = nblk * kDiaRows * nol, nmask = nblk * kDiaRows + 2;
+  hipError_t e1 = hipMalloc((void **)&ex->sym_valL, sizeof(double) * nval);
+  hipError_t e2 = hipMalloc((void **)&ex->sym_diag, sizeof(double) * (size_t)n);
+  hipError_t e3 = hipMalloc((void **)&ex->sym_mask, sizeof(unsigned short) * nmask);
+  if (e1 != hipSuccess || e2 != hipSuccess || e3 != hipSuccess) {
+    (void)hipGetLastError();
+    if (e1 == hipSuccess) (void)hipFree(ex->sym_valL);
+    if (e2 == hipSuccess) (void)hipFree(ex->sym_diag);
+    if (e3 == hipSuccess) (void)hipFree(ex->sym_mask);
+    ex->sym_valL = ex->sym_diag = nullptr;
+    ex->sym_mask = nullptr;
+    return PSP_OK;
+  }
+  const size_t last = (nblk - 1) * kDiaRows;
+  PSP_HIP(hipMemsetAsync(ex->sym_valL + last * nol, 0, sizeof(double) * kDiaRows * nol, stream()));
+  PSP_HIP(hipMemsetAsync(ex->sym_mask + last, 0, sizeof(unsigned short) * (kDiaRows + 2), stream()));
+  hipLaunchKernelGGL(w4_sym_tables_kernel, dim3(std::min((n + 255) / 256, 65536)), dim3(256), 0, stream(), n, nol,
+                     ex->dia_val, ex->dia_mask, ex->sym_valL, ex->sym_diag, ex->sym_mask);
+  PSP_LAUNCH_CHECK();
+  PSP_HIP(hipStreamSynchronize(stream()));
+  for (int i = 0; i < 8; ++i) ex->sym_offs.o[i] = i < nol ? ex->dia_offs.o[i] : -1;
+  ex->sym_nol = nol;
+  ex->sym_ms = std::chrono::duration<double, std::milli>(std::chrono::steady_clock::now() - t0).count();
+  ex->sym_tab = 1;
   return PSP_OK;
 }
 
diff --git a/pysparse_amd/csrc/psp_internal.h b/pysparse_amd/csrc/psp_internal.h
--- a/pysparse_amd/csrc/psp_internal.h
+++ b/pysparse_amd/csrc/psp_internal.h
@@ -407,7 +407,11 @@
                         double *q, double *x, double *partials, int *nparts, const PcgDev *dstate, int *available);
 int csr_spmv_scaled_launch(const psp_csr *A, const double *x, double xdiv, double *y, double *partials,
                            int *nparts, int *available, const int *skip = nullptr,
-                           const double *xdiv_dev = nullptr);
+                           const double *xdiv_dev = nullptr, int sym = 0);
+int csr_sym_product_ready(const psp_csr *A, int *ready);
+int csr_spmv_sym_launch(const psp_csr *A, const double *x, double *y, const double *dotv, double *partials,
+                        int *nparts, const int *skip, int use_div = 0, double xdiv = 1.0,
+                        const double *xdiv_dev = nullptr);
 int csr_reordered_view(const psp_csr *A, psp_csr **R, const int **perm, const int **inv);
 int reorder_gather(int n, const int *perm_dev, const double *x, double *xp, const int *skip);
 bool csr_spmv_has_skip(const psp_csr *A);
diff --git a/pysparse_amd/csrc/psp_solvers.hip b/pysparse_amd/csrc/psp_solvers.hip
--- a/pysparse_amd/csrc/psp_solvers.hip
+++ b/pysparse_amd/csrc/psp_solvers.hip
@@ -314,15 +314,19 @@
 }
 
 static int pcg_enqueue_batch(psp_csr *Acsr, const double *dinv, int n, double *x, double *r, double **pp,
-                             double **pp2, double *q, PcgDev *st, double *hist_dev, int batch) {
+                             double **pp2, double *q, PcgDev *st, double *hist_dev, int batch, int sym) {
   Workspace *w;
   PSP_TRY(workspace(&w));
   int np;
   for (int i = 0; i < batch; ++i) {
     int fusedp = 0;
-    PSP_TRY(csr_spmv_pfused_launch(Acsr, r, dinv, *pp, *pp2, q, 0.0, false, w->partials, &np, st, &fusedp));
+    if (!sym)
+      PSP_TRY(csr_spmv_pfused_launch(Acsr, r, dinv, *pp, *pp2, q, 0.0, false, w->partials, &np, st, &fusedp));
     if (fusedp) {
       std::swap(*pp, *pp2);
+    } else if (sym) {
+      PSP_TRY(k_pupdate(n, r, dinv, 0.0, false, *pp, st));
+      PSP_TRY(csr_spmv_sym_launch(Acsr, *pp, q, *pp, w->partials, &np, &st->status));
     } else {
       PSP_TRY(k_pupdate(n, r, dinv, 0.0, false, *pp, st));
       PSP_TRY(csr_spmv_launch(Acsr, *pp, q, *pp, w->partials, &np, &st->status));
@@ -338,7 +342,7 @@
 
 static int pcg_async_loop(psp_csr *Acsr, const double *dinv, int n, double *x, double *r, double *p,
                           double *p2, double *q, double n2b, double tolb, double normr0, double rho0, int maxit,
-                          int *info, int *iter, double *relres, double *hist) {
+                          int *info, int *iter, double *relres, double *hist, int sym) {
   constexpr int kBatch = 16;
   PcgDev *st = nullptr;
   PcgDev *hst = nullptr;
@@ -383,7 +387,7 @@
   hst->maxit = maxit;
   PCG_HIP(hipMemcpyAsync(st, hst, sizeof(PcgDev), hipMemcpyHostToDevice, stream()));
   enqueued = std::min(kBatch, maxit);
-  PCG_TRY(pcg_enqueue_batch(Acsr, dinv, n, x, r, &p, &p2, q, st, hist_dev, enqueued));
+  PCG_TRY(pcg_enqueue_batch(Acsr, dinv, n, x, r, &p, &p2, q, st, hist_dev, enqueued, sym));
   PCG_HIP(hipMemcpyAsync(hst, st, sizeof(PcgDev), hipMemcpyDeviceToHost, stream()));
   PCG_HIP(hipStreamSynchronize(stream()));
   if (!hst->status) {
@@ -393,7 +397,7 @@
         prev = swap_stream(own);
         swapped = true;
         if (hipStreamBeginCapture(own, hipStreamCaptureModeThreadLocal) == hipSuccess) {
-          const int brc = pcg_enqueue_batch(Acsr, dinv, n, x, r, &p, &p2, q, st, hist_dev, kBatch);
+          const int brc = pcg_enqueue_batch(Acsr, dinv, n, x, r, &p, &p2, q, st, hist_dev, kBatch, sym);
           const hipError_t ce = hipStreamEndCapture(own, &graph);
           if (brc != PSP_OK || ce != hipSuccess || graph == nullptr ||
               hipGraphInstantiate(&exec, graph, nullptr, nullptr, 0) != hipSuccess) {
@@ -413,7 +417,7 @@
         PCG_HIP(hipGraphLaunch(exec, stream()));
       } else {
         const int batch = std::max(1, std::min(kBatch, maxit - enqueued));
-        PCG_TRY(pcg_enqueue_batch(Acsr, dinv, n, x, r, &p, &p2, q, st, hist_dev, batch));
+        PCG_TRY(pcg_enqueue_batch(Acsr, dinv, n, x, r, &p, &p2, q, st, hist_dev, batch, sym));
         enqueued += batch;
       }
       PCG_HIP(hipMemcpyAsync(hst, st, sizeof(PcgDev), hipMemcpyDeviceToHost, stream()));
@@ -573,10 +577,11 @@
 
 static int pcg_async_loop_lazy(psp_csr *Acsr, const double *dinv, int n, double *x, double *r, double *p, double *p2,
                                double *q, double n2b, double tolb, double normr0, double rho0, int maxit,
-                               int *info, int *iter, double *relres, double *hist) {
+                               int *info, int *iter, double *relres, double *hist, int sym, int dstream) {
   constexpr int kBatch = 16;
   double *const P[2] = {p, p2};
-  int usepf = (p2 && pcg_lazypf_mode(n)) ? 1 : 0;
+  int usepf = (!sym && p2 && pcg_lazypf_mode(n)) ? 1 : 0;
+  bool pf_noted = false;
   Workspace *w;
   PSP_TRY(workspace(&w));
   PcgDev *st = nullptr, *hst = nullptr;
@@ -630,6 +635,10 @@
         int av = 0;
         PCG_TRY(csr_spmv_pfx_launch(Acsr, r, dinv, P[(e - 1) & 1], P[e & 1], q, x, w->partials, &np, st, &av));
         if (av) {
+          if (!pf_noted) {
+            note_solve("pcg_lazy_pf", 4 + (n > (1 << 21) ? 2 : 0), 56 + 16 * dstream, dstream);
+            pf_noted = true;
+          }
           PCG_TRY(pcg_reduce_xpq(w, stag_parts, np, w->partials, np, w->scal_dev + 8, w->scal_dev, st));
           PCG_TRY(k_r_update(n, 0.0, q, dinv, r, w->partials, &np, st));
           PCG_TRY(pcg_reduce_then<kOpLazyR>(w->partials, np, 2, w->scal_dev + 4, st, hist_dev));
@@ -639,7 +648,10 @@
       }
       PCG_TRY(k_px_update(n, r, dinv, p, x, w->partials, &np_x, st));
       if (!merge_xpq) PCG_TRY(pcg_reduce_then<kOpLazyX>(stag_parts, np_x, 1, w->scal_dev + 8, st, nullptr));
-      PCG_TRY(csr_spmv_launch(Acsr, p, q, p, w->partials, &np, &st->status));
+      if (sym)
+        PCG_TRY(csr_spmv_sym_launch(Acsr, p, q, p, w->partials, &np, &st->status));
+      else
+        PCG_TRY(csr_spmv_launch(Acsr, p, q, p, w->partials, &np, &st->status));
       if (merge_xpq)
         PCG_TRY(pcg_reduce_xpq(w, stag_parts, np_x, w->partials, np, w->scal_dev + 8, w->scal_dev, st));
       else
@@ -801,16 +813,17 @@
       return PSP_OK;
     }
     const int lazy_mode = pcg_lazy_enabled();
+    int sym = 0;
+    PSP_TRY(csr_sym_product_ready(Acsr, &sym));
     const int rl = n > (1 << 21) ? 2 : 0;
     if ((lazy_mode == 2 || (lazy_mode == 1 && (n < (1 << 24) || n >= 3 * (1 << 23)))) && !pcg_graph_enabled()) {
-      const bool pf = p2 && pcg_lazypf_mode(n);
-      note_solve(pf ? "pcg_lazy_pf" : "pcg_lazy", (pf ? 4 : 5) + rl, (pf ? 56 : 64) + 16 * dstream, dstream);
+      note_solve(sym ? "pcg_lazy_sym" : "pcg_lazy", 5 + rl, 64 + 16 * dstream, dstream);
       return pcg_async_loop_lazy(Acsr, dinv, n, x, r, p, p2, q, n2b, tolb, normr, rho_next, maxit, info, iter,
-                                 relres, hist);
-    }
-    note_solve("pcg_eager", 6 + rl, 72 + 16 * dstream, dstream);
+                                 relres, hist, sym, dstream);
+    }
+    note_solve(sym ? "pcg_eager_sym" : "pcg_eager", 6 + rl, 72 + 16 * dstream, dstream);
     return pcg_async_loop(Acsr, dinv, n, x, r, p, p2, q, n2b, tolb, normr, rho_next, maxit, info, iter,
-                          relres, hist);
+                          relres, hist, sym);
   }
   note_solve("pcg_host_scalars", -1, -1, dstream);
 
@@ -1054,7 +1067,7 @@
 static int minres_async_loop(psp_csr *Acsr, const double *dinv, bool hasK, int n, double *x, double *v_hat,
                              double *v_hat_old, double *y, double *y2, double *wv, double *w_old, double *v,
                              double *av, double norm_r0, double beta0, double errtol, int it_max, int *info,
-                             int *iter, double *relres, double *hist) {
+                             int *iter, double *relres, double *hist, int sym) {
   constexpr int kBatch = 16;
   Workspace *w;
   PSP_TRY(workspace(&w));
@@ -1110,7 +1123,7 @@
       const double *vsrc = hasK ? y : v_hat;
       int scaled = 0;
       if (!hasK || y2)
-        MR_TRY(csr_spmv_scaled_launch(Acsr, vsrc, 1.0, av, w->partials, &np, &scaled, &st->skip, &st->beta));
+        MR_TRY(csr_spmv_scaled_launch(Acsr, vsrc, 1.0, av, w->partials, &np, &scaled, &st->skip, &st->beta, sym));
       if (!scaled) {
         if (!v_ready) MR_TRY(k_scale_div(n, vsrc, 1.0, v, st));
         MR_TRY(csr_spmv_launch(Acsr, v, av, v, w->partials, &np, &st->skip));
@@ -1253,9 +1266,11 @@
     note_fallback();
   }
   if (Acsr && kfused && minres_async_enabled() && it_max >= 1 && !(norm_rmr < errtol * norm_r0)) {
-    note_solve("minres_async", 5 + (n > (1 << 21) ? 2 : 0), 88 + 8 * dstream, dstream);
+    int sym = 0;
+    if (!hasK || y2) PSP_TRY(csr_sym_product_ready(Acsr, &sym));
+    note_solve(sym ? "minres_async_sym" : "minres_async", 5 + (n > (1 << 21) ? 2 : 0), 88 + 8 * dstream, dstream);
     return minres_async_loop(Acsr, dinv, hasK, n, x, v_hat, v_hat_old, y, y2, wv, w_old, v, av, norm_r0,
-                             beta, errtol, it_max, info, iter, relres, hist);
+                             beta, errtol, it_max, info, iter, relres, hist, sym);
   }
   note_solve("minres_host_scalars", -1, -1, dstream);
 
diff --git a/pysparse_amd/device.py b/pysparse_amd/device.py
--- a/pysparse_amd/device.py
+++ b/pysparse_amd/device.py
@@ -210,6 +210,11 @@
         v = (C.c_double * 4)()
         check(lib().psp_csr_setup_info(self._h, v))
         return {"reorder_ms": v[0], "products_counted": int(v[1]), "reorder_after": int(v[2]), "reorder_state": int(v[3])}
+
+    def sym_info(self):
+        v = (C.c_double * 4)()
+        check(lib().psp_csr_sym_info(self._h, v))
+        return {"symmetric": int(v[0]) == 1, "tables": int(v[1]), "setup_ms": v[2], "fallbacks": int(v[3])}
 
     def renumbering(self):
         perm = np.empty(self.shape[0], dtype=np.int32)
```

Result: no change. 6141 (median of 2 runs) (-0.0%).
